# filodb/FiloDB

Measured on NVIDIA H100. Metric: samples/s scanned+aggregated (rate over 10M series); % HBM roofline, higher is better.
Workload: dtype f64

## Files before the change

### filodb_b200/csrc/capi.cu

```cuda
#include "../../include/filo_b200.h"
#include "kernels.h"
#include "host_util.h"
#include "scan_tile_layout.h"
#include "scan_wp_layout.h"
#include <cub/cub.cuh>
#include <algorithm>
#include <atomic>
#include <chrono>
#include <cmath>
#include <cstdio>
#include <cstdlib>
#include <cstring>
#include <mutex>
#include <string>
#include <thread>
#include <vector>

using namespace filo;

struct filo_ctx {
  int device = 0;
  filo_cfg cfg{};
  cudaStream_t stream = nullptr;
  int sm_count = 132;
  size_t max_smem_optin = 0;
  std::mutex err_mu;
  std::string err;
  double fn_args[2] = {0.0, 0.0};
  struct ErrSlot { int* h = nullptr; cudaEvent_t ev = nullptr; bool pending = false; };
  std::mutex errslot_mu;
  ErrSlot errslots[16];
  int errslot_next = 0;
  struct ScanSlot {
    uint8_t* h_in = nullptr; size_t h_in_cap = 0;
    int64_t* h_off = nullptr; size_t h_off_cap = 0;
    uint8_t* d_in = nullptr; size_t d_in_cap = 0;
    int64_t* d_off = nullptr; size_t d_off_cap = 0;
    double* d_out = nullptr; size_t d_out_cap = 0;
    void* h_sink = nullptr;
    void* h_gch = nullptr; size_t h_gch_cap = 0;
    void* d_gch = nullptr; size_t d_gch_cap = 0;
    void* h_gs = nullptr; size_t h_gs_cap = 0;
    void* d_gs = nullptr; size_t d_gs_cap = 0;
    uint8_t* d_stage = nullptr; size_t d_stage_cap = 0;
    cudaStream_t stream = nullptr; cudaEvent_t done = nullptr;
  };
  std::mutex scan_mu;
  static constexpr int MAX_SCAN_SLOTS = 8;
  ScanSlot scan[MAX_SCAN_SLOTS];
  struct HostRange { uintptr_t base; size_t bytes; };
  std::vector<HostRange> ranges;
};

struct filo_table {
  int64_t n_series = 0, n_chunks = 0, n_samples = 0, arena_bytes = 0, algorithmic_bytes = 0;
  int32_t max_rows = 0, max_chunks = 0, schema_flags = 0;
  uint32_t max_rec_bytes = 0;
  bool any_nonconst_ts = true;
  bool any_drop = true;
  uint8_t* d_arena = nullptr;
  int64_t* d_rec_off = nullptr;
  int32_t n_groups = 1;
  bool grouped = false;
  int32_t* d_order = nullptr;
  int64_t* d_group_start = nullptr;
  int64_t* d_gis = nullptr;
  int64_t* d_item_begin = nullptr;
  int64_t n_items = 0;
  int seg = 1;
  bool hist = false, hist_exp = false; int hist_nb = 0;
  bool hist_simple = false;
  std::vector<double> hist_tops; double* d_hist_tops = nullptr;
};

static thread_local std::string tl_err;

static int32_t fail(filo_ctx* ctx, int32_t code, const std::string& msg) {
  tl_err = msg;
  if (ctx) { std::lock_guard<std::mutex> g(ctx->err_mu); ctx->err = msg; }
  return code;
}
#define CUDA_TRY(ctx, expr) do { cudaError_t _e = (expr); if (_e != cudaSuccess) \
  return fail(ctx, _e == cudaErrorMemoryAllocation ? FILO_ERR_OOM : FILO_ERR_CUDA, std::string(#expr) + ": " + cudaGetErrorString(_e)); } while (0)

extern "C" {

int32_t filo_last_error(filo_ctx* ctx, char* buf, int32_t len) {
  std::string m;
  if (ctx) { std::lock_guard<std::mutex> g(ctx->err_mu); m = ctx->err; } else m = tl_err;
  if (buf && len > 0) { int n = std::min<int>(len - 1, (int)m.size()); std::memcpy(buf, m.data(), n); buf[n] = 0; }
  return (int32_t)m.size();
}

int32_t filo_ctx_create(int32_t device, const filo_cfg* cfg, filo_ctx** out) {
  if (!out) return fail(nullptr, FILO_ERR_INVALID_ARG, "out is null");
  int ndev = 0;
  cudaError_t e = cudaGetDeviceCount(&ndev);
  if (e != cudaSuccess || ndev == 0)
    return fail(nullptr, FILO_ERR_CUDA, std::string("no CUDA device (no CPU fallback exists): ") + cudaGetErrorString(e));
  if (device < 0 || device >= ndev) return fail(nullptr, FILO_ERR_INVALID_ARG, "bad device ordinal");
  CUDA_TRY(nullptr, cudaSetDevice(device));
  auto* c = new filo_ctx();
  c->device = device;
  if (cfg) c->cfg = *cfg; else { c->cfg.inclusive_range = 1; c->cfg.group_by_cardinality_limit = 0; c->cfg.min_step_ms = 0; c->cfg.max_data_per_shard_query = 0; }
  cudaDeviceProp p; CUDA_TRY(nullptr, cudaGetDeviceProperties(&p, device));
  c->sm_count = p.multiProcessorCount;
  c->max_smem_optin = p.sharedMemPerBlockOptin;
  CUDA_TRY(nullptr, cudaStreamCreateWithFlags(&c->stream, cudaStreamNonBlocking));
  {
    cudaMemPool_t pool = nullptr;
    if (cudaDeviceGetDefaultMemPool(&pool, device) == cudaSuccess && pool) {
      uint64_t thr = ~0ull;
      cudaMemPoolSetAttribute(pool, cudaMemPoolAttrReleaseThreshold, &thr);
    }
    cudaGetLastError();
  }
  *out = c;
  return FILO_OK;
}

int32_t filo_ctx_set_fn_args(filo_ctx* ctx, double arg0, double arg1) {
  if (!ctx) return fail(nullptr, FILO_ERR_INVALID_ARG, "ctx is null");
  ctx->fn_args[0] = arg0; ctx->fn_args[1] = arg1;
  return FILO_OK;
}

void filo_ctx_destroy(filo_ctx* ctx) {
  if (!ctx) return;
  cudaSetDevice(ctx->device);
  if (ctx->stream) cudaStreamDestroy(ctx->stream);
  for (auto& sl : ctx->errslots) { if (sl.ev) { cudaEventSynchronize(sl.ev); cudaEventDestroy(sl.ev); } if (sl.h) cudaFreeHost(sl.h); }
  for (auto& r : ctx->ranges) cudaHostUnregister((void*)r.base);
  for (auto& sl : ctx->scan) {
    if (sl.stream) cudaStreamSynchronize(sl.stream);
    cudaFreeHost(sl.h_in); cudaFreeHost(sl.h_off); cudaFreeHost(sl.h_sink); cudaFree(sl.d_in); cudaFree(sl.d_off); cudaFree(sl.d_out);
    cudaFreeHost(sl.h_gch); cudaFreeHost(sl.h_gs); cudaFree(sl.d_gch); cudaFree(sl.d_gs); cudaFree(sl.d_stage);
    if (sl.done) cudaEventDestroy(sl.done);
    if (sl.stream) cudaStreamDestroy(sl.stream);
  }
  delete ctx;
}

void filo_table_free(filo_ctx* ctx, filo_table* t) {
  if (!t) return;
  if (ctx) cudaSetDevice(ctx->device);
  cudaFree(t->d_arena); cudaFree(t->d_rec_off); cudaFree(t->d_order); cudaFree(t->d_group_start);
  cudaFree(t->d_gis); cudaFree(t->d_item_begin); cudaFree(t->d_hist_tops);
  delete t;
}

int32_t filo_table_get_info(const filo_table* t, filo_table_info* o) {
  if (!t || !o) return FILO_ERR_INVALID_ARG;
  o->n_series = t->n_series; o->n_chunks = t->n_chunks; o->n_samples = t->n_samples; o->arena_bytes = t->arena_bytes;
  o->algorithmic_bytes = t->algorithmic_bytes; o->max_rows_per_series = t->max_rows; o->max_chunks_per_series = t->max_chunks;
  o->n_groups = t->n_groups; o->schema_flags = t->schema_flags; o->hist_buckets = t->hist ? t->hist_nb : 0; o->reserved = 0;
  return FILO_OK;
}

int32_t filo_num_windows(int64_t start, int64_t step, int64_t end) {
  if (step <= 0) step = 1;
  if (end < start) return 1;
  return (int32_t)((end - start) / step) + 1;
}

}

static bool hist_v2_enabled() { const char* e = getenv("FILO_HIST_V2"); return !(e && e[0] == '0'); }

static int32_t build_groups_new(filo_ctx* ctx, filo_table* t, const int32_t* d_group_ids, int32_t n_groups);
static int32_t build_groups(filo_ctx* ctx, filo_table* t, const int32_t* d_group_ids , int32_t n_groups) {
  int32_t* o_order = t->d_order; int64_t* o_gs = t->d_group_start; int64_t* o_gis = t->d_gis; int64_t* o_ib = t->d_item_begin;
  const int32_t o_ng = t->n_groups; const bool o_grouped = t->grouped; const int64_t o_items = t->n_items; const int o_seg = t->seg;
  t->d_order = nullptr; t->d_group_start = t->d_gis = t->d_item_begin = nullptr;
  const int32_t rc = build_groups_new(ctx, t, d_group_ids, n_groups);
  if (rc != FILO_OK) {
    cudaFree(t->d_order); cudaFree(t->d_group_start); cudaFree(t->d_gis); cudaFree(t->d_item_begin);
    t->d_order = o_order; t->d_group_start = o_gs; t->d_gis = o_gis; t->d_item_begin = o_ib;
    t->n_groups = o_ng; t->grouped = o_grouped; t->n_items = o_items; t->seg = o_seg;
    return rc;
  }
  cudaFree(o_order); cudaFree(o_gs); cudaFree(o_gis); cudaFree(o_ib);
  return FILO_OK;
}
static int32_t build_groups_new(filo_ctx* ctx, filo_table* t, const int32_t* d_group_ids , int32_t n_groups) {
  cudaStream_t s = ctx->stream;
  const int64_t S = t->n_series;
  if (n_groups <= 0) n_groups = 1;
  t->n_groups = n_groups;
  t->grouped = d_group_ids != nullptr;
  int64_t target_items = (int64_t)ctx->sm_count * 64 * 4;
  int64_t seg_cap = 256;
  if (t->hist && hist_v2_enabled()) { target_items = (int64_t)ctx->sm_count * 2 * 6; seg_cap = 4096; }
  int64_t seg = S / std::max<int64_t>(target_items, 1);
  t->seg = (int)std::min<int64_t>(std::max<int64_t>(seg, 1), seg_cap);
  CUDA_TRY(ctx, cudaMalloc(&t->d_group_start, (size_t)(n_groups + 1) * 8));
  CUDA_TRY(ctx, cudaMalloc(&t->d_gis, (size_t)(n_groups + 1) * 8));
  if (t->grouped && S > 0) {
    int32_t *keys_out = nullptr, *vals_in = nullptr;
    CUDA_TRY(ctx, cudaMalloc(&t->d_order, (size_t)S * 4));
    CUDA_TRY(ctx, cudaMalloc(&keys_out, (size_t)S * 4));
    CUDA_TRY(ctx, cudaMalloc(&vals_in, (size_t)S * 4));
    CUDA_TRY(ctx, launch_iota(vals_in, S, s));
    size_t tmp_bytes = 0;
    int end_bit = 1; while ((1ll << end_bit) < n_groups && end_bit < 31) ++end_bit;
    cub::DeviceRadixSort::SortPairs(nullptr, tmp_bytes, d_group_ids, keys_out, vals_in, t->d_order, (int)S, 0, end_bit, s);
    void* tmp = nullptr; CUDA_TRY(ctx, cudaMalloc(&tmp, tmp_bytes + 16));
    CUDA_TRY(ctx, cub::DeviceRadixSort::SortPairs(tmp, tmp_bytes, d_group_ids, keys_out, vals_in, t->d_order, (int)S, 0, end_bit, s));
    CUDA_TRY(ctx, launch_group_bounds(keys_out, S, n_groups, t->d_group_start, s));
    CUDA_TRY(ctx, cudaStreamSynchronize(s));
    cudaFree(tmp); cudaFree(keys_out); cudaFree(vals_in);
  } else {
    std::vector<int64_t> gs(n_groups + 1, S); gs[0] = 0;
    CUDA_TRY(ctx, cudaMemcpyAsync(t->d_group_start, gs.data(), gs.size() * 8, cudaMemcpyHostToDevice, s));
    CUDA_TRY(ctx, cudaStreamSynchronize(s));
  }
  int64_t* d_cnt = nullptr; CUDA_TRY(ctx, cudaMalloc(&d_cnt, (size_t)(n_groups + 1) * 8));
  CUDA_TRY(ctx, cudaMemsetAsync(d_cnt, 0, (size_t)(n_groups + 1) * 8, s));
  CUDA_TRY(ctx, launch_group_item_count(t->d_group_start, n_groups, t->seg, d_cnt, s));
  size_t tmp_bytes = 0;
  cub::DeviceScan::ExclusiveSum(nullptr, tmp_bytes, d_cnt, t->d_gis, n_groups + 1, s);
  void* tmp = nullptr; CUDA_TRY(ctx, cudaMalloc(&tmp, tmp_bytes + 16));
  CUDA_TRY(ctx, cub::DeviceScan::ExclusiveSum(tmp, tmp_bytes, d_cnt, t->d_gis, n_groups + 1, s));
  int64_t n_items = 0;
  CUDA_TRY(ctx, cudaMemcpyAsync(&n_items, t->d_gis + n_groups, 8, cudaMemcpyDeviceToHost, s));
  CUDA_TRY(ctx, cudaStreamSynchronize(s));
  t->n_items = n_items;
  CUDA_TRY(ctx, cudaMalloc(&t->d_item_begin, (size_t)(n_items + 1) * 8));
  CUDA_TRY(ctx, launch_fill_items(t->d_group_start, t->d_gis, n_groups, t->seg, n_items, S, t->d_item_begin, s));
  CUDA_TRY(ctx, cudaStreamSynchronize(s));
  cudaFree(tmp); cudaFree(d_cnt);
  return FILO_OK;
}

int32_t filo_internal_finish_table(filo_ctx* ctx, filo_table* t, const int32_t* d_group_ids, int32_t n_groups) {
  return build_groups(ctx, t, d_group_ids, n_groups);
}
filo_table* filo_internal_new_table() { return new filo_table(); }
void filo_internal_set_arena(filo_table* t, uint8_t* d_arena, int64_t* d_rec_off, int64_t n_series, int64_t n_chunks, int64_t n_samples,
                             int64_t arena_bytes, int64_t algorithmic_bytes, int32_t max_rows, int32_t max_chunks, int32_t schema_flags) {
  t->d_arena = d_arena; t->d_rec_off = d_rec_off; t->n_series = n_series; t->n_chunks = n_chunks; t->n_samples = n_samples;
  t->arena_bytes = arena_bytes; t->algorithmic_bytes = algorithmic_bytes; t->max_rows = max_rows; t->max_chunks = max_chunks;
  t->schema_flags = schema_flags;
}
void filo_internal_set_layout(filo_table* t, uint32_t max_rec_bytes, bool any_nonconst_ts, bool any_drop) {
  t->max_rec_bytes = max_rec_bytes; t->any_nonconst_ts = any_nonconst_ts; t->any_drop = any_drop;
}
cudaStream_t filo_internal_stream(filo_ctx* ctx) { return ctx->stream; }
int filo_internal_device(filo_ctx* ctx) { return ctx->device; }
int32_t filo_internal_fail(filo_ctx* ctx, int32_t code, const char* msg) { return fail(ctx, code, msg); }

namespace {

struct GatherChunk {
  uint64_t ts_src, val_src;
  int64_t start_time, end_time;
  int32_t num_rows, ts_bytes, val_bytes, val_len;
  int32_t drop_patch, pad;
};
struct GatherSeries { uint32_t rec_bytes, n_chunks, n_rows, flags; int64_t first_chunk; };

struct VecInfo { const uint8_t* p; int32_t total; int32_t len; bool drop_patch; bool drop; bool hist = false; };

inline int32_t rd32(const uint8_t* p) { int32_t v; std::memcpy(&v, p, 4); return v; }
inline int64_t rd64(const uint8_t* p) { int64_t v; std::memcpy(&v, p, 8); return v; }

inline bool inner_ok(const uint8_t* in, int32_t& len, int32_t outer_total) {
  const int32_t inner_bytes = rd32(in);
  if (inner_bytes < 4 || (int64_t)20 + 4 + inner_bytes > outer_total) return false;
  int nbits = in[6] & 0x7f; bool sgn = in[6] & 0x80; int bs = in[7] & 0x3f;
  bool ok = sgn ? (nbits == 32 || nbits == 16 || nbits == 8) : (nbits == 32 || nbits == 16 || nbits == 8 || nbits == 4 || nbits == 2);
  if (!ok) return false;
  len = ((rd32(in) - 4) * 8 + (bs != 0 ? bs - 8 : 0)) / nbits;
  return true;
}

int classify_ts(const uint8_t* v, VecInfo& o) {
  int wire = (uint16_t)(v[4] | (v[5] << 8));
  if (wire == WIRE_MASKED) { v = v + rd32(v + 8); wire = (uint16_t)(v[4] | (v[5] << 8)); if (wire == WIRE_MASKED) return FILO_ERR_CORRUPT_VECTOR; }
  o.p = v; o.total = rd32(v) + 4; o.drop_patch = false; o.drop = false;
  if (o.total < 8 || o.total > (1 << 28)) return FILO_ERR_CORRUPT_VECTOR;
  if (wire == WIRE_DDV_CONST) { if (o.total != 24) return FILO_ERR_CORRUPT_VECTOR; o.len = rd32(v + 8); }
  else if (wire == WIRE_RAW64) o.len = (rd32(v) - 4) / 8;
  else if (wire == WIRE_DDV) { if (o.total < 28 || !inner_ok(v + 20, o.len, o.total)) return FILO_ERR_CORRUPT_VECTOR; }
  else return FILO_ERR_CORRUPT_VECTOR;
  return (o.total >= 8 && o.len >= 0) ? 0 : FILO_ERR_CORRUPT_VECTOR;
}
int classify_val(const uint8_t* v, VecInfo& o) {
  int wire = (uint16_t)(v[4] | (v[5] << 8));
  const bool outer_drop = (v[7] & 0x80) != 0;
  bool masked = false;
  if (wire == WIRE_MASKED) { masked = true; v = v + rd32(v + 8); wire = (uint16_t)(v[4] | (v[5] << 8)); if (wire == WIRE_MASKED) return FILO_ERR_CORRUPT_VECTOR; }
  o.p = v; o.total = rd32(v) + 4; o.drop_patch = masked; o.drop = outer_drop;
  if (o.total < 8 || o.total > (1 << 28)) return FILO_ERR_CORRUPT_VECTOR;
  if (wire == WIRE_RAW64) o.len = (rd32(v) - 4) / 8;
  else if (wire == WIRE_DDV_CONST) { if (o.total != 24) return FILO_ERR_CORRUPT_VECTOR; o.len = rd32(v + 8); }
  else if (wire == WIRE_DDV) { if (o.total < 28 || !inner_ok(v + 20, o.len, o.total)) return FILO_ERR_CORRUPT_VECTOR; }
  else if (wire == WIRE_XOR) {
    o.len = rd32(v + XOR_OFF_N);
    int ng = (uint16_t)(v[12] | (v[13] << 8)), po = (uint16_t)(v[14] | (v[15] << 8));
    if (o.len <= 0 || ng != (o.len - 1 + 7) / 8 || po < 16 + 2 * ng || (po & 7) || po + 8 > o.total) return FILO_ERR_CORRUPT_VECTOR;
  } else if (wire == WIRE_H_SECTDELTA || wire == WIRE_H_SIMPLE) {
    if (masked || o.total < 13) return FILO_ERR_CORRUPT_VECTOR;
    o.len = (uint16_t)(v[6] | (v[7] << 8)); o.drop = false; o.hist = true;
    const int fmt = v[8], defBytes = (uint16_t)(v[9] | (v[10] << 8));
    if (o.len > 0 && (!(fmt == 3 || fmt == 4 || fmt == 5 || fmt == 9) || 11 + defBytes > o.total || (fmt == 9 && defBytes != 16)))
      return (fmt == 8 || fmt == 0x0a || fmt == 0x10 || fmt == 9) ? FILO_ERR_UNSUPPORTED : FILO_ERR_CORRUPT_VECTOR;
  } else if (wire == WIRE_H_EXP_SIMPLE) return FILO_ERR_UNSUPPORTED;
  else return FILO_ERR_CORRUPT_VECTOR;
  return (o.total >= 8 && o.len >= 0) ? 0 : FILO_ERR_CORRUPT_VECTOR;
}

struct SeriesPlan { uint32_t rec_bytes; uint32_t n_chunks; uint32_t n_rows; uint32_t flags; };

struct LoadIn { int64_t n_series; const int32_t* n_chunks; const uint64_t* addrs; const int64_t* chunk_base ; int32_t ts_col, val_col;
                GatherChunk* gc_out = nullptr; int64_t gc_base = 0; const std::vector<filo_ctx::HostRange>* ranges = nullptr;
                int64_t cb0 = 0; };
struct PlanTotals { int64_t chunks = 0, samples = 0, alg = 0; int32_t maxrows = 0, maxch = 0; uint32_t max_rec = 0, f_or = 0, f_and = ~0u;
// ... 155 lines not shown
  CUDA_TRY(ctx, cudaMemcpy(t->d_hist_tops, t->hist_tops.data(), (size_t)nb * 8, cudaMemcpyHostToDevice));
  return FILO_OK;
}
static int32_t filo_load_series_impl(filo_ctx* ctx, int64_t n_series, const int32_t* n_chunks, const uint64_t* addrs,
                                    int32_t ts_col, int32_t val_col, const int32_t* group_ids, int32_t n_groups,
                                    int32_t schema_flags, filo_table** out) {
  if (!ctx || !out || n_series < 0 || (n_series > 0 && (!n_chunks || !addrs)) || ts_col < 0 || val_col < 0)
    return fail(ctx, FILO_ERR_INVALID_ARG, "filo_load_series: bad arguments");
  if (group_ids && n_groups <= 0) return fail(ctx, FILO_ERR_INVALID_ARG, "group_ids given but n_groups <= 0");
  if (group_ids && ctx->cfg.group_by_cardinality_limit > 0 && n_groups > ctx->cfg.group_by_cardinality_limit)
    return fail(ctx, FILO_ERR_QUERY_LIMIT, "Query exceeded group-by cardinality limit");
  CUDA_TRY(ctx, cudaSetDevice(ctx->device));
  std::vector<int64_t> chunk_base((size_t)n_series + 1, 0);
  for (int64_t i = 0; i < n_series; ++i) {
    if (n_chunks[i] < 0) return fail(ctx, FILO_ERR_INVALID_ARG, "negative n_chunks");
    chunk_base[i + 1] = chunk_base[i] + n_chunks[i];
  }
  std::vector<SeriesPlan> plan((size_t)n_series);
  const LoadIn in{n_series, n_chunks, addrs, chunk_base.data(), ts_col, val_col};
  PlanTotals tot; int64_t err_series = -1;
  if (const int err_code = plan_all(in, plan, tot, err_series)) {
    const char* what = err_code == FILO_ERR_UNSUPPORTED ? "chunks of a series are not in increasing time order (unsupported on the device path)"
                                                       : "CorruptVector: unknown or inconsistent BinaryVector wire format";
    return fail(ctx, err_code, std::string(what) + " at series " + std::to_string(err_series));
  }
  std::vector<int64_t> rec_off((size_t)n_series + 1, 0);
  for (int64_t i = 0; i < n_series; ++i) rec_off[i + 1] = rec_off[i] + plan[i].rec_bytes;
  const int64_t arena_bytes = rec_off[n_series];
  if (ctx->cfg.max_data_per_shard_query > 0 && tot.alg > ctx->cfg.max_data_per_shard_query)
    return fail(ctx, FILO_ERR_QUERY_LIMIT, "raw data bytes scanned exceeds max-data-per-shard-query");
  if (tot.hist_def && tot.any_scalar) return fail(ctx, FILO_ERR_UNSUPPORTED, "histogram and scalar value vectors in one table");
  if (tot.hist_mismatch) return fail(ctx, FILO_ERR_UNSUPPORTED, "histogram bucket schemes differ inside the table (unsupported on the device path)");
  struct LoadGuard {
    filo_table* t = nullptr; uint8_t* d_arena = nullptr; int64_t* d_rec_off = nullptr; uint8_t* slab[2] = {nullptr, nullptr}; cudaEvent_t ev[2] = {nullptr, nullptr};
    bool owns_table = true;
    ~LoadGuard() {
      for (int b = 0; b < 2; ++b) { if (ev[b]) { cudaEventSynchronize(ev[b]); cudaEventDestroy(ev[b]); } if (slab[b]) cudaFreeHost(slab[b]); }
      if (owns_table) { cudaFree(d_arena); cudaFree(d_rec_off); delete t; }
    }
  } lg;
  lg.t = new filo_table();
  filo_table*& t = lg.t; uint8_t*& d_arena = lg.d_arena; int64_t*& d_rec_off = lg.d_rec_off;
  CUDA_TRY(ctx, cudaMalloc(&d_arena, (size_t)arena_bytes + 64));
  CUDA_TRY(ctx, cudaMalloc(&d_rec_off, (size_t)(n_series + 1) * 8));
  CUDA_TRY(ctx, cudaMemsetAsync(d_arena + arena_bytes, 0, 64, ctx->stream));
  CUDA_TRY(ctx, cudaMemcpyAsync(d_rec_off, rec_off.data(), (size_t)(n_series + 1) * 8, cudaMemcpyHostToDevice, ctx->stream));
  const size_t SLAB = std::min<size_t>((size_t)256 << 20, std::max<size_t>((size_t)arena_bytes, 1 << 16));
  uint8_t** slab = lg.slab; cudaEvent_t* ev = lg.ev;
  for (int b = 0; b < 2; ++b) { CUDA_TRY(ctx, cudaHostAlloc(&slab[b], SLAB + (1 << 20), cudaHostAllocDefault)); CUDA_TRY(ctx, cudaEventCreateWithFlags(&ev[b], cudaEventDisableTiming)); }
  int64_t s0 = 0; int which = 0;
  while (s0 < n_series) {
    int64_t s1 = s0; const int64_t base = rec_off[s0];
    while (s1 < n_series && (size_t)(rec_off[s1 + 1] - base) <= SLAB) ++s1;
    if (s1 == s0) {
      const size_t need = (size_t)plan[s0].rec_bytes;
      CUDA_TRY(ctx, cudaEventSynchronize(ev[which]));
      cudaFreeHost(slab[which]); slab[which] = nullptr;
      CUDA_TRY(ctx, cudaHostAlloc(&slab[which], need + (1 << 20), cudaHostAllocDefault)); s1 = s0 + 1;
    }
    CUDA_TRY(ctx, cudaEventSynchronize(ev[which]));
    uint8_t* dst0 = slab[which];
    host_pool().run(s1 - s0, [&](int, int64_t b, int64_t e) {
      for (int64_t ii = b; ii < e; ++ii) { const int64_t i = s0 + ii; fill_record(in, i, plan[(size_t)i], dst0 + (rec_off[i] - base)); }
    });
    CUDA_TRY(ctx, cudaMemcpyAsync(d_arena + base, dst0, (size_t)(rec_off[s1] - base), cudaMemcpyHostToDevice, ctx->stream));
    CUDA_TRY(ctx, cudaEventRecord(ev[which], ctx->stream));
    which ^= 1; s0 = s1;
  }
  CUDA_TRY(ctx, cudaStreamSynchronize(ctx->stream));
  lg.owns_table = false;
  filo_internal_set_arena(t, d_arena, d_rec_off, n_series, tot.chunks, tot.samples, arena_bytes + (n_series + 1) * 8, tot.alg, tot.maxrows, tot.maxch, schema_flags);
  filo_internal_set_layout(t, tot.max_rec, n_series > 0 && !(tot.f_and & REC_ALL_TS_CONST), (tot.f_or & REC_ANY_DROP) != 0);
  if (tot.hist_def) {
    const int32_t rch = filo_internal_set_hist(ctx, t, tot.hist_def);
    if (rch != FILO_OK) { filo_table_free(ctx, t); return rch; }
    t->hist_simple = tot.hist_simple;
  }
  int32_t* d_gid = nullptr;
  if (group_ids && n_series > 0) {
    for (int64_t i = 0; i < n_series; ++i) if (group_ids[i] < 0 || group_ids[i] >= n_groups) { filo_table_free(ctx, t); return fail(ctx, FILO_ERR_INVALID_ARG, "group id out of range"); }
    CUDA_TRY(ctx, cudaMalloc(&d_gid, (size_t)n_series * 4));
    CUDA_TRY(ctx, cudaMemcpy(d_gid, group_ids, (size_t)n_series * 4, cudaMemcpyHostToDevice));
  }
  int32_t rc = build_groups(ctx, t, d_gid, group_ids ? n_groups : 1);
  cudaFree(d_gid);
  if (rc) { filo_table_free(ctx, t); return rc; }
  *out = t;
  return FILO_OK;
}
extern "C" int32_t filo_load_series(filo_ctx* ctx, int64_t n_series, const int32_t* n_chunks, const uint64_t* addrs,
                                    int32_t ts_col, int32_t val_col, const int32_t* group_ids, int32_t n_groups,
                                    int32_t schema_flags, filo_table** out) {
  try { return filo_load_series_impl(ctx, n_series, n_chunks, addrs, ts_col, val_col, group_ids, n_groups, schema_flags, out); }
  catch (const std::bad_alloc&) { return fail(ctx, FILO_ERR_OOM, "filo_load_series: host allocation failed"); }
  catch (const std::exception& e) { return fail(ctx, FILO_ERR_INVALID_ARG, std::string("filo_load_series: ") + e.what()); }
}

extern "C" int32_t filo_table_set_groups(filo_ctx* ctx, filo_table* t, const int32_t* group_ids, int32_t n_groups) {
  if (!ctx || !t) return fail(ctx, FILO_ERR_INVALID_ARG, "null");
  CUDA_TRY(ctx, cudaSetDevice(ctx->device));
  if (group_ids && ctx->cfg.group_by_cardinality_limit > 0 && n_groups > ctx->cfg.group_by_cardinality_limit)
    return fail(ctx, FILO_ERR_QUERY_LIMIT, "Query exceeded group-by cardinality limit");
  int32_t* d_gid = nullptr;
  if (group_ids && t->n_series > 0) {
    for (int64_t i = 0; i < t->n_series; ++i) if (group_ids[i] < 0 || group_ids[i] >= n_groups) return fail(ctx, FILO_ERR_INVALID_ARG, "group id out of range");
    CUDA_TRY(ctx, cudaMalloc(&d_gid, (size_t)t->n_series * 4));
    CUDA_TRY(ctx, cudaMemcpy(d_gid, group_ids, (size_t)t->n_series * 4, cudaMemcpyHostToDevice));
  }
  int32_t rc = build_groups(ctx, t, d_gid, group_ids ? n_groups : 1);
  cudaFree(d_gid);
  return rc;
}

extern "C" int64_t filo_table_read_record(filo_ctx* ctx, const filo_table* t, int64_t series, uint8_t* out, int64_t cap) {
  if (!ctx || !t || series < 0 || series >= t->n_series) return fail(ctx, FILO_ERR_INVALID_ARG, "bad series");
  cudaSetDevice(ctx->device);
  int64_t off[2];
  if (cudaMemcpy(off, t->d_rec_off + series, 16, cudaMemcpyDeviceToHost) != cudaSuccess) return fail(ctx, FILO_ERR_CUDA, "read rec_off");
  int64_t n = off[1] - off[0];
  if (n > cap) return -n;
  if (cudaMemcpy(out, t->d_arena + off[0], (size_t)n, cudaMemcpyDeviceToHost) != cudaSuccess) return fail(ctx, FILO_ERR_CUDA, "read record");
  return n;
}

namespace {
__device__ __forceinline__ uint32_t rec_used_vectors(const uint8_t* r) {
  const RecordHeader h = *reinterpret_cast<const RecordHeader*>(r);
  const uint32_t v0 = (uint32_t)sizeof(RecordHeader) + 32u * h.n_chunks;
  if (h.n_chunks == 0) return 0;
  const ChunkEntry& e = reinterpret_cast<const ChunkEntry*>(r + sizeof(RecordHeader))[h.n_chunks - 1];
  const uint32_t vt = *reinterpret_cast<const uint32_t*>(r + e.val_off) + 4u;
  return align_up(e.val_off + vt, 8) - v0;
}
__global__ void append_size_kernel(const uint8_t* __restrict__ ar_o, const int64_t* __restrict__ off_o, const uint8_t* __restrict__ ar_d, const int64_t* __restrict__ off_d,
                                   int64_t n, int64_t* __restrict__ sz) {
  const int64_t i = (int64_t)blockIdx.x * blockDim.x + threadIdx.x;
  if (i < n) {
    const uint8_t* ro = ar_o + off_o[i]; const uint8_t* rd = ar_d + off_d[i];
    const uint32_t nn = reinterpret_cast<const RecordHeader*>(ro)->n_chunks + reinterpret_cast<const RecordHeader*>(rd)->n_chunks;
    sz[i] = (int64_t)align_up((uint32_t)sizeof(RecordHeader) + 32u * nn + rec_used_vectors(ro) + rec_used_vectors(rd), 16);
  }
  if (i == n) sz[i] = 0;
}
__global__ void __launch_bounds__(256) append_merge_kernel(const uint8_t* __restrict__ ar_o, const int64_t* __restrict__ off_o, const uint8_t* __restrict__ ar_d,
                                                           const int64_t* __restrict__ off_d, const int64_t* __restrict__ off_n, int64_t n,
                                                           uint8_t* __restrict__ ar_n, unsigned int* __restrict__ stats) {
  const int lane = threadIdx.x & 31;
  const int64_t i = ((int64_t)blockIdx.x * blockDim.x + threadIdx.x) >> 5;
  if (i >= n) return;
  const uint8_t* ro = ar_o + off_o[i]; const uint8_t* rd = ar_d + off_d[i]; uint8_t* rn = ar_n + off_n[i];
  const RecordHeader ho = *reinterpret_cast<const RecordHeader*>(ro), hd = *reinterpret_cast<const RecordHeader*>(rd);
  const uint32_t no = ho.n_chunks, nd = hd.n_chunks, nn = no + nd;
  const uint32_t vo0 = (uint32_t)sizeof(RecordHeader) + 32u * no, vd0 = (uint32_t)sizeof(RecordHeader) + 32u * nd, vn0 = (uint32_t)sizeof(RecordHeader) + 32u * nn;
  const uint32_t Lo = rec_used_vectors(ro), Ld = rec_used_vectors(rd);
  const uint32_t rec_bytes = align_up(vn0 + Lo + Ld, 16);
  if (lane == 0) {
    RecordHeader hn; hn.rec_bytes = rec_bytes; hn.n_chunks = nn; hn.n_rows = ho.n_rows + hd.n_rows;
    hn.flags = ((ho.flags & hd.flags) & REC_ALL_TS_CONST) | ((ho.flags | hd.flags) & ~REC_ALL_TS_CONST);
    *reinterpret_cast<RecordHeader*>(rn) = hn;
    atomicMax(&stats[0], hn.rec_bytes); atomicMax(&stats[1], hn.n_rows); atomicMax(&stats[2], nn);
    if (no && nd) {
      const ChunkEntry& lo = reinterpret_cast<const ChunkEntry*>(ro + sizeof(RecordHeader))[no - 1];
      const ChunkEntry& fd = reinterpret_cast<const ChunkEntry*>(rd + sizeof(RecordHeader))[0];
      if (fd.start_time < lo.start_time || fd.end_time < lo.end_time) atomicAdd(&stats[3], 1u);
    }
    if ((vn0 + Lo + Ld) & 8u) *reinterpret_cast<uint64_t*>(rn + vn0 + Lo + Ld) = 0ull;
  }
  for (uint32_t c = lane; c < nn; c += 32) {
    ChunkEntry e;
    if (c < no) { e = reinterpret_cast<const ChunkEntry*>(ro + sizeof(RecordHeader))[c]; e.ts_off += 32u * nd; e.val_off += 32u * nd; }
    else { e = reinterpret_cast<const ChunkEntry*>(rd + sizeof(RecordHeader))[c - no]; e.ts_off += 32u * no + Lo; e.val_off += 32u * no + Lo; e.row_base += ho.n_rows; }
    reinterpret_cast<ChunkEntry*>(rn + sizeof(RecordHeader))[c] = e;
  }
  const uint64_t* so = reinterpret_cast<const uint64_t*>(ro + vo0); uint64_t* dn = reinterpret_cast<uint64_t*>(rn + vn0);
  for (uint32_t q = lane; q < Lo / 8; q += 32) dn[q] = so[q];
  const uint64_t* sd = reinterpret_cast<const uint64_t*>(rd + vd0); dn = reinterpret_cast<uint64_t*>(rn + vn0 + Lo);
  for (uint32_t q = lane; q < Ld / 8; q += 32) dn[q] = sd[q];
}
}

static int32_t filo_table_append_impl(filo_ctx* ctx, filo_table* t, const int32_t* n_chunks, const uint64_t* chunk_info_addrs, int32_t ts_col, int32_t val_col) {
  if (!ctx || !t || !n_chunks || !chunk_info_addrs) return fail(ctx, FILO_ERR_INVALID_ARG, "filo_table_append: null argument");
  if (t->hist) return fail(ctx, FILO_ERR_UNSUPPORTED, "filo_table_append: histogram tables are rebuilt with filo_load_series");
  const int64_t S = t->n_series;
  filo_table* d = nullptr;
  { const int32_t rc = filo_load_series(ctx, S, n_chunks, chunk_info_addrs, ts_col, val_col, nullptr, 0, t->schema_flags, &d); if (rc != FILO_OK) return rc; }
  struct FreeT { filo_ctx* c; filo_table* t; ~FreeT() { filo_table_free(c, t); } } guard{ctx, d};
  if (d->hist) return fail(ctx, FILO_ERR_UNSUPPORTED, "filo_table_append: histogram vectors");
  CUDA_TRY(ctx, cudaSetDevice(ctx->device));
  cudaStream_t s = ctx->stream;
  int64_t *d_sz = nullptr, *d_off = nullptr; unsigned int* d_stats = nullptr; void* tmp = nullptr; uint8_t* d_arena = nullptr;
  struct FreeD { std::vector<void*> p; ~FreeD() { for (void* x : p) cudaFree(x); } } tmps;
  CUDA_TRY(ctx, cudaMalloc(&d_sz, (size_t)(S + 1) * 8)); tmps.p.push_back(d_sz);
  CUDA_TRY(ctx, cudaMalloc(&d_off, (size_t)(S + 1) * 8));
  CUDA_TRY(ctx, cudaMalloc(&d_stats, 16)); tmps.p.push_back(d_stats);
  CUDA_TRY(ctx, cudaMemsetAsync(d_stats, 0, 16, s));
  append_size_kernel<<<(unsigned)((S + 1 + 255) / 256), 256, 0, s>>>(t->d_arena, t->d_rec_off, d->d_arena, d->d_rec_off, S, d_sz);
  size_t tmp_bytes = 0;
  cub::DeviceScan::ExclusiveSum(nullptr, tmp_bytes, d_sz, d_off, (int)(S + 1), s);
  if (cudaMalloc(&tmp, tmp_bytes + 16) != cudaSuccess) { cudaFree(d_off); return fail(ctx, FILO_ERR_OOM, "filo_table_append: scan storage"); }
  tmps.p.push_back(tmp);
  if (cub::DeviceScan::ExclusiveSum(tmp, tmp_bytes, d_sz, d_off, (int)(S + 1), s) != cudaSuccess) { cudaFree(d_off); return fail(ctx, FILO_ERR_CUDA, "filo_table_append: scan"); }
  int64_t arena_bytes = 0;
  if (cudaMemcpyAsync(&arena_bytes, d_off + S, 8, cudaMemcpyDeviceToHost, s) != cudaSuccess || cudaStreamSynchronize(s) != cudaSuccess) { cudaFree(d_off); return fail(ctx, FILO_ERR_CUDA, "filo_table_append: sizes"); }
  if (cudaMalloc(&d_arena, (size_t)arena_bytes + 64) != cudaSuccess) { cudaFree(d_off); return fail(ctx, FILO_ERR_OOM, "filo_table_append: the new arena does not fit beside the old one"); }
  cudaMemsetAsync(d_arena + arena_bytes, 0, 64, s);
  if (S > 0) append_merge_kernel<<<(unsigned)((S * 32 + 255) / 256), 256, 0, s>>>(t->d_arena, t->d_rec_off, d->d_arena, d->d_rec_off, d_off, S, d_arena, d_stats);
  unsigned int st[4] = {0, 0, 0, 0};
  cudaError_t e = cudaGetLastError();
  if (e == cudaSuccess) e = cudaMemcpyAsync(st, d_stats, 16, cudaMemcpyDeviceToHost, s);
  if (e == cudaSuccess) e = cudaStreamSynchronize(s);
  if (e != cudaSuccess) { cudaFree(d_off); cudaFree(d_arena); return fail(ctx, FILO_ERR_CUDA, std::string("filo_table_append: ") + cudaGetErrorString(e)); }
  if (st[3]) { cudaFree(d_off); cudaFree(d_arena); return fail(ctx, FILO_ERR_UNSUPPORTED, "filo_table_append: new chunks must follow the resident ones in time (unsupported on the device path)"); }
  cudaFree(t->d_arena); cudaFree(t->d_rec_off);
  t->d_arena = d_arena; t->d_rec_off = d_off;
  t->n_chunks += d->n_chunks; t->n_samples += d->n_samples; t->algorithmic_bytes += d->algorithmic_bytes;
  t->arena_bytes = arena_bytes + (S + 1) * 8;
  t->max_rec_bytes = st[0]; t->max_rows = (int32_t)st[1]; t->max_chunks = (int32_t)st[2];
  t->any_nonconst_ts = t->any_nonconst_ts || (d->n_chunks > 0 && d->any_nonconst_ts); t->any_drop = t->any_drop || d->any_drop;
  return FILO_OK;
}
extern "C" int32_t filo_table_append(filo_ctx* ctx, filo_table* t, const int32_t* n_chunks, const uint64_t* chunk_info_addrs, int32_t ts_col, int32_t val_col) {
  try { return filo_table_append_impl(ctx, t, n_chunks, chunk_info_addrs, ts_col, val_col); }
  catch (const std::bad_alloc&) { return fail(ctx, FILO_ERR_OOM, "filo_table_append: host allocation failed"); }
  catch (const std::exception& e) { return fail(ctx, FILO_ERR_INVALID_ARG, std::string("filo_table_append: ") + e.what()); }
}

extern "C" int64_t filo_table_read_arena(filo_ctx* ctx, const filo_table* t, int64_t first, int64_t n, uint8_t* out, int64_t cap,
                                         int64_t* rec_off_out) {
  if (!ctx || !t || first < 0 || n < 0 || first + n > t->n_series || !rec_off_out) return fail(ctx, FILO_ERR_INVALID_ARG, "bad range");
  cudaSetDevice(ctx->device);
  if (cudaMemcpy(rec_off_out, t->d_rec_off + first, (size_t)(n + 1) * 8, cudaMemcpyDeviceToHost) != cudaSuccess)
    return fail(ctx, FILO_ERR_CUDA, "read rec_off");
  const int64_t base = rec_off_out[0], bytes = rec_off_out[n] - base;
  for (int64_t i = 0; i <= n; ++i) rec_off_out[i] -= base;
  if (bytes > cap || !out) return -bytes;
  if (bytes > 0 && cudaMemcpy(out, t->d_arena + base, (size_t)bytes, cudaMemcpyDeviceToHost) != cudaSuccess)
    return fail(ctx, FILO_ERR_CUDA, "read arena");
  return bytes;
}

namespace {
struct Temp {
  cudaStream_t s; std::vector<void*> ptrs;
  explicit Temp(cudaStream_t st) : s(st) {}
  ~Temp() { for (void* p : ptrs) cudaFreeAsync(p, s); }
  cudaError_t alloc(void** p, size_t bytes) { cudaError_t e = cudaMallocAsync(p, bytes ? bytes : 16, s); if (e == cudaSuccess) ptrs.push_back(*p); return e; }
};
}

namespace {
struct AsyncSink { int herr[4]; unsigned long long hc[2]; int64_t launches; };
}
static int32_t query_device_impl(filo_ctx* ctx, const filo_table* t, int32_t fn, int64_t start, int64_t step, int64_t end, int64_t window,
                                 int32_t agg, int32_t k, int32_t flags, void* d_out_values, void* d_out_aux, void* cuda_stream,
                                 filo_stats* stats, AsyncSink* sink);
extern "C" int32_t filo_query_device(filo_ctx* ctx, const filo_table* t, int32_t fn, int64_t start, int64_t step, int64_t end, int64_t window,
                                     int32_t agg, int32_t k, int32_t flags, void* d_out_values, void* d_out_aux, void* cuda_stream,
                                     filo_stats* stats) {
  return query_device_impl(ctx, t, fn, start, step, end, window, agg, k, flags, d_out_values, d_out_aux, cuda_stream, stats, nullptr);
}
namespace {
struct EventPair {
  cudaEvent_t e0 = nullptr, e1 = nullptr;
  ~EventPair() { if (e0) cudaEventDestroy(e0); if (e1) cudaEventDestroy(e1); }
};
}
static int32_t report_device_error(filo_ctx* ctx, const int herr[4], int64_t series_base);
static int32_t poll_async_errors(filo_ctx* ctx, bool wait) {
  std::lock_guard<std::mutex> g(ctx->errslot_mu);
  int32_t rc = FILO_OK;
  for (auto& sl : ctx->errslots) {
    if (!sl.pending) continue;
    cudaError_t e = wait ? cudaEventSynchronize(sl.ev) : cudaEventQuery(sl.ev);
    if (e == cudaErrorNotReady) { cudaGetLastError(); continue; }
    sl.pending = false;
    if (e != cudaSuccess) { if (rc == FILO_OK) rc = fail(ctx, FILO_ERR_CUDA, std::string("asynchronous query: ") + cudaGetErrorString(e)); continue; }
    if (sl.h[0] && rc == FILO_OK) rc = report_device_error(ctx, sl.h, 0);
  }
  return rc;
}
static int32_t push_async_error(filo_ctx* ctx, const int* d_err, cudaStream_t s) {
  std::lock_guard<std::mutex> g(ctx->errslot_mu);
  filo_ctx::ErrSlot& sl = ctx->errslots[ctx->errslot_next];
  ctx->errslot_next = (ctx->errslot_next + 1) % 16;
  if (!sl.h) { CUDA_TRY(ctx, cudaMallocHost((void**)&sl.h, 16)); CUDA_TRY(ctx, cudaEventCreateWithFlags(&sl.ev, cudaEventDisableTiming)); }
  if (sl.pending) {
    CUDA_TRY(ctx, cudaEventSynchronize(sl.ev)); sl.pending = false;
    if (sl.h[0]) return report_device_error(ctx, sl.h, 0);
  }
  CUDA_TRY(ctx, cudaMemcpyAsync(sl.h, d_err, 16, cudaMemcpyDeviceToHost, s));
  CUDA_TRY(ctx, cudaEventRecord(sl.ev, s));
  sl.pending = true;
  return FILO_OK;
}
extern "C" int32_t filo_ctx_check(filo_ctx* ctx) {
  if (!ctx) return fail(nullptr, FILO_ERR_INVALID_ARG, "ctx is null");
  return poll_async_errors(ctx, true);
}
static int32_t report_device_error(filo_ctx* ctx, const int herr[4], int64_t series_base) {
  if (herr[0] == 5)
    return fail(ctx, FILO_ERR_UNSUPPORTED, "histogram series with more chunks / sections / rows in range than the device path holds, at series " +
                std::to_string(series_base + ((int64_t)herr[1] | ((int64_t)herr[2] << 31))));
  const char* what = herr[0] == 4 ? "series needs more decode scratch than the table statistics promised" : "CorruptVector on device";
  return fail(ctx, FILO_ERR_CORRUPT_VECTOR, std::string(what) + " (code " + std::to_string(herr[0]) + ") at series " +
              std::to_string(series_base + ((int64_t)herr[1] | ((int64_t)herr[2] << 31))));
}
static int32_t query_device_impl(filo_ctx* ctx, const filo_table* t, int32_t fn, int64_t start, int64_t step, int64_t end, int64_t window,
                                 int32_t agg, int32_t k, int32_t flags, void* d_out_values, void* d_out_aux, void* cuda_stream,
                                 filo_stats* stats, AsyncSink* sink) {
  if (!ctx || !t || !d_out_values) return fail(ctx, FILO_ERR_INVALID_ARG, "filo_query: null argument");
  if (fn < FILO_FN_LAST || fn > FILO_FN_PRESENT_OVER_TIME) return fail(ctx, FILO_ERR_INVALID_ARG, "unknown range function");
  if (t->hist) return fail(ctx, FILO_ERR_UNSUPPORTED, "histogram table: use filo_query_hist");
  const bool long_values = (t->schema_flags & FILO_SCHEMA_LONG_VALUES) != 0;
  if (long_values && !fn_long_column_ok(fn)) return fail(ctx, FILO_ERR_UNSUPPORTED, "no chunked range function for this function on a Long column");
  if (fn == FILO_FN_HOLT_WINTERS) {
    if (!(ctx->fn_args[0] >= 0 && ctx->fn_args[0] <= 1)) return fail(ctx, FILO_ERR_INVALID_ARG, "Sf should be in between 0 and 1");
    if (!(ctx->fn_args[1] >= 0 && ctx->fn_args[1] <= 1)) return fail(ctx, FILO_ERR_INVALID_ARG, "tf should be in between 0 and 1");
  }
  if (agg < FILO_AGG_NONE || agg > FILO_AGG_GROUP) return fail(ctx, FILO_ERR_INVALID_ARG, "unknown aggregation operator");
  if (start > end) return fail(ctx, FILO_ERR_INVALID_ARG, "start should be <= end");
  if (!(start == end || step > 0)) return fail(ctx, FILO_ERR_INVALID_ARG, "step should be > 0 for range query");
  if (start < end && step < ctx->cfg.min_step_ms) return fail(ctx, FILO_ERR_BAD_QUERY, "step should be at least min-step");
  const int64_t adjustedStep = step > 0 ? step : step + 1;
  const bool isLast = (fn == FILO_FN_LAST || fn == FILO_FN_TIMESTAMP);
  if (window <= 0) { if (isLast) window = 5 * 60 * 1000 + 1; else return fail(ctx, FILO_ERR_INVALID_ARG, "Need positive window lengths to apply range function"); }
  if ((agg == FILO_AGG_TOPK || agg == FILO_AGG_BOTTOMK) && (k <= 0 || k > FILO_MAX_TOPK)) return fail(ctx, FILO_ERR_INVALID_ARG, "topk/bottomk k must be in [1, 32]");
  if ((agg == FILO_AGG_TOPK || agg == FILO_AGG_BOTTOMK || agg == FILO_AGG_AVG) && !d_out_aux && !(agg == FILO_AGG_AVG && !(flags & FILO_Q_PARTIAL)))
    return fail(ctx, FILO_ERR_INVALID_ARG, "out_aux required");
  if ((flags & FILO_Q_PARTIAL) && agg != FILO_AGG_NONE && agg != FILO_AGG_TOPK && agg != FILO_AGG_BOTTOMK && !d_out_aux)
    return fail(ctx, FILO_ERR_INVALID_ARG, "partial aggregates need out_aux (counts)");
  CUDA_TRY(ctx, cudaSetDevice(ctx->device));
  { const int32_t prc = poll_async_errors(ctx, false); if (prc != FILO_OK) return prc; }
  cudaStream_t s = cuda_stream ? (cudaStream_t)cuda_stream : ctx->stream;
  QueryParams q{};
  q.start = start; q.step = adjustedStep; q.end = end; q.window = window; q.T = filo_num_windows(start, adjustedStep, end);
  q.fn = fn; q.cumulative = (t->schema_flags & FILO_SCHEMA_CUMULATIVE) ? 1 : 0; q.inclusive = ctx->cfg.inclusive_range ? 1 : 0;
  q.long_values = long_values ? 1 : 0; q.p0 = ctx->fn_args[0]; q.p1 = ctx->fn_args[1];
  const bool need_corr = (fn == FILO_FN_RATE || fn == FILO_FN_INCREASE) && q.cumulative;
  const bool fused = (agg != FILO_AGG_NONE && agg != FILO_AGG_TOPK && agg != FILO_AGG_BOTTOMK);
  const bool moments = agg_moments(agg);
  const int scan_op = moments ? AGG_SUM : agg == FILO_AGG_GROUP ? AGG_COUNT : agg;

  Temp tmp(s);
  int* d_err = nullptr; unsigned long long* d_counters = nullptr;
  CUDA_TRY(ctx, tmp.alloc((void**)&d_err, 16)); CUDA_TRY(ctx, tmp.alloc((void**)&d_counters, 16));
  CUDA_TRY(ctx, cudaMemsetAsync(d_err, 0, 16, s)); CUDA_TRY(ctx, cudaMemsetAsync(d_counters, 0, 16, s));
  EventPair evp;
  if (stats) { CUDA_TRY(ctx, cudaEventCreate(&evp.e0)); CUDA_TRY(ctx, cudaEventCreate(&evp.e1)); }
  cudaEvent_t& e0 = evp.e0; cudaEvent_t& e1 = evp.e1;

  const uint32_t acc_bytes = fused ? align_up((uint32_t)q.T * (moments ? 20u : 12u), 128) : 0;
  const bool need_corr2 = need_corr && t->any_drop;
  uint32_t scratch2 = align_up((uint32_t)t->max_chunks * (uint32_t)CHUNK_DESC_BYTES, 16) +
                      ((uint32_t)t->max_rows + (uint32_t)t->max_chunks * 8u) * 8u * (1u + (t->any_nonconst_ts ? 1u : 0u) + (need_corr2 ? 1u : 0u));
  scratch2 = align_up(scratch2 + 16, 128);
  const uint32_t rec_cap = align_up(t->max_rec_bytes + 16, 128);
  const size_t per_warp2 = v2_smem_per_warp(rec_cap, scratch2, acc_bytes);
  const char* force_env = std::getenv("FILO_KERNEL");
  const std::string force = force_env ? force_env : "";
  const size_t smem_cap = std::min<size_t>(ctx->max_smem_optin, 227 * 1024);
  const bool use_v2 = force != "v1" && t->max_rec_bytes > 0 && per_warp2 * FAST_WARPS + 1024 <= smem_cap;
  const int64_t work = fused ? t->n_items : t->n_series;
  int64_t launches = 0;
  uint8_t* gscratch = nullptr;
  ScanLaunch L{t->d_arena, t->d_rec_off, t->n_series, q, nullptr, 0, 0, d_counters, d_err, 1, s};
  uint32_t rec_cap_used = 0;
  if (use_v2) {
    const size_t cta_smem = per_warp2 * FAST_WARPS + 1024;
    const int ctas_per_sm = (int)std::max<size_t>(1, std::min<size_t>(64 / FAST_WARPS, (size_t)(228 * 1024) / cta_smem));
    L.grid = (int)std::max<int64_t>(1, std::min<int64_t>((work + FAST_WARPS - 1) / FAST_WARPS, (int64_t)ctx->sm_count * ctas_per_sm));
    L.scratch_bytes = scratch2; L.use_smem = 1; rec_cap_used = rec_cap;
  } else {
    uint32_t scratch = align_up((uint32_t)t->max_chunks * (uint32_t)CHUNK_DESC_BYTES, 16) + (uint32_t)t->max_rows * 8u * (need_corr ? 3u : 2u);
    scratch = align_up(scratch + 16, 16);
    const size_t cta_smem = (size_t)(scratch + acc_bytes) * SCAN_WARPS;
    const int use_smem = cta_smem <= std::min<size_t>(ctx->max_smem_optin, 200 * 1024);
    int ctas_per_sm = 16;
    if (use_smem) ctas_per_sm = (int)std::max<size_t>(1, std::min<size_t>(16, (size_t)(220 * 1024) / std::max<size_t>(cta_smem + 1024, 1)));
    L.grid = (int)std::max<int64_t>(1, std::min<int64_t>((work + SCAN_WARPS - 1) / SCAN_WARPS, (int64_t)ctx->sm_count * ctas_per_sm));
    if (!use_smem) CUDA_TRY(ctx, tmp.alloc((void**)&gscratch, (size_t)L.grid * SCAN_WARPS * (scratch + acc_bytes)));
    L.gscratch = gscratch; L.scratch_bytes = scratch; L.use_smem = use_smem;
  }
  const int fn_cls = fn_class_of(fn, q.cumulative, q.long_values);
  const uint64_t wrows = (uint64_t)(q.window / q.step) + 1;
  TileSmem TL{};
  bool use_tile = false;
  if (use_v2 && force != "v2" && fn_cls == CLASS_SUM && t->n_series > 0) {
    TL = tile_layout(t->max_rec_bytes, (uint32_t)t->max_rows, (uint32_t)q.T, (uint32_t)std::min<uint64_t>(2 * wrows, 1u << 20) + 16);
    if (((size_t)TL.total + 1024) * 2 > (size_t)228 * 1024) TL = tile_layout(t->max_rec_bytes, (uint32_t)t->max_rows, (uint32_t)q.T, 16);
    use_tile = (size_t)TL.total + 1024 <= smem_cap;
  }
  WpSmem WL{};
  bool use_wp = false;
  if (use_tile && force != "v3" && wrows <= 4096 && t->max_chunks > 0) {
    const bool alias = wp_max_items((uint32_t)t->max_chunks, (uint32_t)q.T, (uint32_t)wrows) <= 64;
    WL = wp_layout(t->max_rec_bytes, (uint32_t)t->max_rows, (uint32_t)t->max_chunks, (uint32_t)q.T, (uint32_t)wrows, alias);
    WL.warps = (uint32_t)std::min<size_t>(smem_cap / WL.per_warp, alias ? WP_MAX_WARPS_ALIAS : WP_MAX_WARPS);
    const WpSmem WL2 = wp_layout(t->max_rec_bytes, (uint32_t)t->max_rows, (uint32_t)t->max_chunks, (uint32_t)q.T, (uint32_t)wrows, alias, true);
    if (smem_cap / WL2.per_warp >= (size_t)WP_MAX_WARPS) { WL = WL2; WL.warps = WP_MAX_WARPS; }
    use_wp = WL.warps >= 4;
  }
  WpCtrSmem WC{};
  bool use_wp_ctr = false;
  if (use_v2 && force != "v2" && force != "v3" && fn_cls == CLASS_COUNTER && t->n_series > 0 && t->max_chunks > 0 &&
      (!fused || q.T <= TILE_AGG_ACC * TILE_THREADS) && wp_ctr_tile_footprint_ok(t->max_rec_bytes, (uint32_t)t->max_rows, (uint32_t)q.T, smem_cap)) {
    WC = wp_ctr_layout(t->max_rec_bytes, (uint32_t)t->max_rows, (uint32_t)t->max_chunks, (uint32_t)q.T, fused, t->any_nonconst_ts, moments);
    const size_t w = std::min<size_t>((smem_cap - sizeof(TileCtrTab) * (TILE_CTR_TABMAX + 1) - 64) / WC.per_warp, WC.tsr != 0 ? 16 : WP_CTR_MAX_WARPS);
    WC.warps = (uint32_t)w; WC.tab = (uint32_t)(WC.per_warp * w);
    use_wp_ctr = w >= 4;
  }
  auto run_per_series = [&](double* outp) -> int32_t {
    if (use_tile || use_wp_ctr) {
      int64_t* d_list = nullptr; unsigned long long* d_cnt = nullptr;
      CUDA_TRY(ctx, tmp.alloc((void**)&d_list, (size_t)t->n_series * 8));
      CUDA_TRY(ctx, tmp.alloc((void**)&d_cnt, 16));
      CUDA_TRY(ctx, cudaMemsetAsync(d_cnt, 0, 16, s));
      ScanLaunch LT = L;
      static const bool dbg = std::getenv("FILO_DEBUG_SYNC") != nullptr;
      if (use_wp) {
        LT.grid = (int)std::max<int64_t>(1, std::min<int64_t>((t->n_series + WL.warps - 1) / WL.warps, (int64_t)ctx->sm_count));
        CUDA_TRY(ctx, launch_scan_wp(LT, outp, WL, d_list, d_cnt));
      } else if (use_wp_ctr) {
        LT.grid = (int)std::max<int64_t>(1, std::min<int64_t>((t->n_series + WC.warps - 1) / WC.warps, (int64_t)ctx->sm_count));
        CUDA_TRY(ctx, launch_scan_wp_ctr(LT, outp, WC, d_list, d_cnt));
      } else {
        const int ctas_per_sm = ((size_t)TL.total + 1024) * 2 <= (size_t)228 * 1024 ? 2 : 1;
        const int64_t n_tiles = (t->n_series + TILE_NS - 1) / TILE_NS;
        LT.grid = (int)std::max<int64_t>(1, std::min<int64_t>(n_tiles, (int64_t)ctx->sm_count * ctas_per_sm));
        if (dbg) { fprintf(stderr, "[filo] tile kernel fn=%d T=%d grid=%d smem=%u pitch=%u\n", fn, q.T, LT.grid, TL.total, TL.vals_pitch); fflush(stderr); }
        CUDA_TRY(ctx, launch_scan_tile(LT, outp, TL, d_list, d_cnt));
      }
      if (dbg) { CUDA_TRY(ctx, cudaStreamSynchronize(s)); fprintf(stderr, "[filo] tile kernel done\n"); fflush(stderr); }
      ScanLaunch LF = L; LF.list = d_list; LF.list_count = d_cnt;
      CUDA_TRY(ctx, launch_scan_series_v2(LF, outp, rec_cap_used));
      if (dbg) { CUDA_TRY(ctx, cudaStreamSynchronize(s)); fprintf(stderr, "[filo] fallback kernel done\n"); fflush(stderr); }
      launches += 2;
    } else {
      CUDA_TRY(ctx, use_v2 ? launch_scan_series_v2(L, outp, rec_cap_used) : launch_scan_series(L, outp));
      launches += 1;
    }
    return FILO_OK;
  };
  if (stats) CUDA_TRY(ctx, cudaEventRecord(e0, s));
  if (agg == FILO_AGG_NONE) {
    { int32_t rc = run_per_series((double*)d_out_values); if (rc) return rc; }
  } else if (!fused) {
    double* per = nullptr;
    CUDA_TRY(ctx, tmp.alloc((void**)&per, (size_t)t->n_series * q.T * 8));
// ... 311 lines not shown
      int32_t rg = FILO_OK;
      if (!use_gather) rg = grow_pinned(ctx, sl.h_in, sl.h_in_cap, B.bytes + 64);
      else {
        rg = grow_pinned(ctx, sl.h_gch, sl.h_gch_cap, (size_t)(B.chunks + 1) * sizeof(GatherChunk));
        if (!rg) rg = grow_device(ctx, sl.d_gch, sl.d_gch_cap, (size_t)(B.chunks + 1) * sizeof(GatherChunk));
        if (!rg) rg = grow_pinned(ctx, sl.h_gs, sl.h_gs_cap, (size_t)(nb + 1) * sizeof(GatherSeries));
        if (!rg) rg = grow_device(ctx, sl.d_gs, sl.d_gs_cap, (size_t)(nb + 1) * sizeof(GatherSeries));
      }
      if (!rg) rg = grow_pinned(ctx, sl.h_off, sl.h_off_cap, (size_t)(nb + 1) * 8);
      if (!rg) rg = grow_device(ctx, sl.d_in, sl.d_in_cap, B.bytes + 64);
      if (!rg) rg = grow_device(ctx, sl.d_off, sl.d_off_cap, (size_t)(nb + 1) * 8);
      if (!rg) rg = grow_device(ctx, sl.d_out, sl.d_out_cap, (size_t)nb * (size_t)std::max(T, 1) * 8);
      if (rg) { rc = rg; break; }
    }
    if (trace_path) {
      TraceRow tr{nb, B.bytes, ms_since(t_begin), {nullptr, nullptr, nullptr, nullptr}};
      for (auto& e : tr.ev) cudaEventCreate(&e);
      if (!trace_t0) { cudaEventCreate(&trace_t0); cudaEventRecord(trace_t0, sl.stream); }
      cudaEventRecord(tr.ev[0], sl.stream);
      trace.push_back(tr);
    }
    const auto t_f0 = now();
    sl.h_off[0] = 0;
    for (int64_t j = 0; j < nb; ++j) sl.h_off[j + 1] = sl.h_off[j] + plan[(size_t)(B.s0 + j - c0)].rec_bytes;
    cudaError_t ce = cudaSuccess;
    if (use_gather) {
      GatherSeries* gs = reinterpret_cast<GatherSeries*>(sl.h_gs); GatherChunk* gc = reinterpret_cast<GatherChunk*>(sl.h_gch);
      int64_t cb = 0;
      for (int64_t j = 0; j < nb; ++j) { const SeriesPlan& p = plan[(size_t)(B.s0 + j - c0)]; gs[j] = GatherSeries{p.rec_bytes, p.n_chunks, p.n_rows, p.flags, cb}; cb += p.n_chunks; }
      std::atomic<uint64_t> span_lo{~0ull}, span_hi{0};
      host_pool().run(nb, [&](int, int64_t b, int64_t e) {
        uint64_t lo = ~0ull, hi = 0;
        for (int64_t j = b; j < e; ++j) {
          const int64_t i = B.s0 + j; GatherChunk* o = gc + gs[j].first_chunk;
          const GatherChunk* src = gc_walk.data() + (chunk_base[(size_t)(i - c0)] - in.gc_base);
          for (uint32_t jj = 0; jj < gs[j].n_chunks; ++jj) {
            const GatherChunk g = src[jj];
            *o++ = g;
            lo = std::min(lo, std::min(g.ts_src, g.val_src));
            hi = std::max(hi, std::max(g.ts_src + (uint64_t)g.ts_bytes, g.val_src + (uint64_t)g.val_bytes));
          }
        }
        uint64_t cur = span_lo.load(); while (lo < cur && !span_lo.compare_exchange_weak(cur, lo)) {}
        cur = span_hi.load(); while (hi > cur && !span_hi.compare_exchange_weak(cur, hi)) {}
      });
      t_fill += ms_since(t_f0);
      int64_t rebase = 0;
      {
        static const bool no_span = [] { const char* e = std::getenv("FILO_SCAN_SPAN"); return e && e[0] == '0'; }();
        const uint64_t lo = span_lo.load() & ~(uint64_t)15, hi = span_hi.load();
        if (!no_span && hi > lo && (hi - lo) <= (uint64_t)B.bytes + (uint64_t)B.bytes / 2 + (1u << 20) && in_ranges(reinterpret_cast<const uint8_t*>((uintptr_t)lo), (size_t)(hi - lo))) {
          if (int32_t rcg = grow_device(ctx, sl.d_stage, sl.d_stage_cap, (size_t)(hi - lo) + 64)) return rcg;
          ce = cudaMemcpyAsync(sl.d_stage, reinterpret_cast<const void*>((uintptr_t)lo), (size_t)(hi - lo), cudaMemcpyHostToDevice, sl.stream);
          rebase = (int64_t)((uint64_t)(uintptr_t)sl.d_stage - lo);
        }
      }
      if (ce == cudaSuccess)
      ce = cudaMemcpyAsync(sl.d_gs, sl.h_gs, (size_t)nb * sizeof(GatherSeries), cudaMemcpyHostToDevice, sl.stream);
      if (ce == cudaSuccess) ce = cudaMemcpyAsync(sl.d_gch, sl.h_gch, (size_t)B.chunks * sizeof(GatherChunk), cudaMemcpyHostToDevice, sl.stream);
      if (ce == cudaSuccess) ce = cudaMemcpyAsync(sl.d_off, sl.h_off, (size_t)(nb + 1) * 8, cudaMemcpyHostToDevice, sl.stream);
      if (ce == cudaSuccess) {
        const int grid = (int)std::max<int64_t>(1, std::min<int64_t>((nb + 7) / 8, (int64_t)ctx->sm_count * 8));
        gather_records_kernel<<<grid, 256, 0, sl.stream>>>(reinterpret_cast<const GatherSeries*>(sl.d_gs), reinterpret_cast<const GatherChunk*>(sl.d_gch),
                                                           sl.d_off, nb, sl.d_in, rebase);
        ce = cudaGetLastError();
      }
      if (ce == cudaSuccess) ce = cudaMemsetAsync(sl.d_in + B.bytes, 0, 64, sl.stream);
    } else {
      host_pool().run(nb, [&](int, int64_t b, int64_t e) {
        for (int64_t j = b; j < e; ++j) fill_record(in, B.s0 + j, plan[(size_t)(B.s0 + j - c0)], sl.h_in + sl.h_off[j]);
      });
      std::memset(sl.h_in + B.bytes, 0, 64);
      t_fill += ms_since(t_f0);
      ce = cudaMemcpyAsync(sl.d_in, sl.h_in, B.bytes + 64, cudaMemcpyHostToDevice, sl.stream);
      if (ce == cudaSuccess) ce = cudaMemcpyAsync(sl.d_off, sl.h_off, (size_t)(nb + 1) * 8, cudaMemcpyHostToDevice, sl.stream);
    }
    const auto t_e0 = now();
    if (ce != cudaSuccess) { rc = fail(ctx, FILO_ERR_CUDA, std::string("scan H2D: ") + cudaGetErrorString(ce)); break; }
    if (trace_path) cudaEventRecord(trace.back().ev[1], sl.stream);
    filo_table view;
    view.n_series = nb; view.d_arena = sl.d_in; view.d_rec_off = sl.d_off; view.max_rows = tot.maxrows; view.max_chunks = tot.maxch;
    view.max_rec_bytes = tot.max_rec; view.any_nonconst_ts = !(tot.f_and & REC_ALL_TS_CONST); view.any_drop = (tot.f_or & REC_ANY_DROP) != 0;
    view.schema_flags = schema_flags; view.n_groups = 1; view.grouped = false;
    rc = query_device_impl(ctx, &view, fn, start, step, end, window, FILO_AGG_NONE, 0, 0, sl.d_out, nullptr, sl.stream, nullptr,
                           reinterpret_cast<AsyncSink*>(sl.h_sink));
    if (rc != FILO_OK) break;
    if (trace_path) cudaEventRecord(trace.back().ev[2], sl.stream);
    ce = cudaMemcpyAsync(out_values + (size_t)B.s0 * T, sl.d_out, (size_t)nb * T * 8, cudaMemcpyDeviceToHost, sl.stream);
    if (trace_path) cudaEventRecord(trace.back().ev[3], sl.stream);
    if (ce == cudaSuccess) ce = cudaEventRecord(sl.done, sl.stream);
    if (ce != cudaSuccess) { rc = fail(ctx, FILO_ERR_CUDA, std::string("scan D2H: ") + cudaGetErrorString(ce)); break; }
    fl[si].s0 = B.s0;
    t_enq += ms_since(t_e0);
    acc.h2d_bytes += (int64_t)B.bytes + (nb + 1) * 8 + (use_gather ? (int64_t)(nb * sizeof(GatherSeries) + B.chunks * sizeof(GatherChunk)) : 0); acc.d2h_bytes += nb * (int64_t)T * 8;
  }
  }
  for (int i = 0; i < NSLOT; ++i) { const int32_t r2 = retire(i); if (rc == FILO_OK) rc = r2; }
  if (rc != FILO_OK) { for (int i = 0; i < NSLOT; ++i) if (ctx->scan[i].stream) cudaStreamSynchronize(ctx->scan[i].stream); return rc; }
  if (trace_path) {
    if (FILE* f = std::fopen(trace_path, "w")) {
      std::fprintf(f, "batch,series,bytes,host_enqueue_ms,start_ms,h2d_done_ms,kernels_done_ms,d2h_done_ms\n");
      for (size_t i = 0; i < trace.size(); ++i) {
        float t[4] = {0, 0, 0, 0};
        for (int j = 0; j < 4; ++j) cudaEventElapsedTime(&t[j], trace_t0, trace[i].ev[j]);
        std::fprintf(f, "%zu,%lld,%zu,%.3f,%.3f,%.3f,%.3f,%.3f\n", i, (long long)trace[i].nb, trace[i].bytes, trace[i].host_ms, t[0], t[1], t[2], t[3]);
      }
      std::fclose(f);
    }
    for (auto& r : trace) for (auto& e : r.ev) cudaEventDestroy(e);
    if (trace_t0) cudaEventDestroy(trace_t0);
  }
  if (timing) fprintf(stderr, "[filo] scan_series: %lld series, %zu batches, total %.1f ms: plan %.1f, fill %.1f, enqueue %.1f, slot waits %.1f\n",
                      (long long)n_series, n_batches, ms_since(t_begin), t_plan, t_fill, t_enq, t_retire);
  if (stats) *stats = acc;
  return FILO_OK;
}
extern "C" int32_t filo_scan_series(filo_ctx* ctx, int64_t n_series, const int32_t* n_chunks, const uint64_t* addrs,
                                    int32_t ts_col, int32_t val_col, int32_t schema_flags,
                                    int32_t fn, int64_t start, int64_t step, int64_t end, int64_t window,
                                    double* out_values, filo_stats* stats) {
  try { return filo_scan_series_impl(ctx, n_series, n_chunks, addrs, ts_col, val_col, schema_flags, fn, start, step, end, window, out_values, stats); }
  catch (const std::bad_alloc&) { return fail(ctx, FILO_ERR_OOM, "filo_scan_series: host allocation failed"); }
  catch (const std::exception& e) { return fail(ctx, FILO_ERR_INVALID_ARG, std::string("filo_scan_series: ") + e.what()); }
}


static int32_t hist_query_impl(filo_ctx* ctx, const filo_table* t, int32_t fn, int64_t start, int64_t step, int64_t end, int64_t window,
                               int32_t agg, double quantile, double* out_values, double* out_quantile, void* cuda_stream, filo_stats* stats, bool host_out) {
  if (!ctx || !t || (!out_values && !out_quantile)) return fail(ctx, FILO_ERR_INVALID_ARG, "filo_query_hist: null argument");
  if (!t->hist) return fail(ctx, FILO_ERR_INVALID_ARG, "filo_query_hist: not a histogram table");
  if (agg != FILO_AGG_NONE && agg != FILO_AGG_SUM) return fail(ctx, FILO_ERR_UNSUPPORTED, "histogram aggregates: sum only");
  if (!(fn == FILO_FN_RATE || fn == FILO_FN_INCREASE || fn == FILO_FN_SUM_OVER_TIME || fn == FILO_FN_LAST))
    return fail(ctx, FILO_ERR_UNSUPPORTED, "histogram range functions on the device path: rate, increase, sum_over_time, last");
  if (start > end) return fail(ctx, FILO_ERR_INVALID_ARG, "start should be <= end");
  if (!(start == end || step > 0)) return fail(ctx, FILO_ERR_INVALID_ARG, "step should be > 0 for range query");
  if (start < end && step < ctx->cfg.min_step_ms) return fail(ctx, FILO_ERR_BAD_QUERY, "step should be at least min-step");
  const bool last = fn == FILO_FN_LAST;
  if (window <= 0) { if (last) window = 5 * 60 * 1000 + 1; else return fail(ctx, FILO_ERR_INVALID_ARG, "Need positive window lengths to apply range function"); }
  CUDA_TRY(ctx, cudaSetDevice(ctx->device));
  { const int32_t prc = poll_async_errors(ctx, false); if (prc != FILO_OK) return prc; }
  cudaStream_t s = cuda_stream ? (cudaStream_t)cuda_stream : ctx->stream;
  const int64_t adjustedStep = step > 0 ? step : step + 1;
  QueryParams q{};
  q.start = start; q.step = adjustedStep; q.end = end; q.window = window; q.T = filo_num_windows(start, adjustedStep, end);
  q.fn = fn; q.cumulative = (t->schema_flags & FILO_SCHEMA_CUMULATIVE) ? 1 : 0; q.inclusive = ctx->cfg.inclusive_range ? 1 : 0;
  const int nb = t->hist_nb, T = q.T;
  const bool fused = agg == FILO_AGG_SUM;
  const bool pq = !fused && out_quantile;
  const size_t smem = hist_smem_bytes(t->max_rows, nb, T, fused || pq, t->max_rec_bytes);
  const size_t smem2 = hist2_smem_bytes(t->max_rows, nb, t->max_rec_bytes);
  const bool v2 = hist_v2_enabled() && ((q.cumulative && (fn == FILO_FN_RATE || fn == FILO_FN_INCREASE)) || (last && !t->hist_simple)) && T <= 32 * 512 && nb <= 64 &&
                  smem2 + 1024 <= std::min<size_t>(ctx->max_smem_optin, 227 * 1024) && (fused || pq || last);
  if (!(v2 && !fused) && smem + 2048 > std::min<size_t>(ctx->max_smem_optin, 227 * 1024))
    return fail(ctx, FILO_ERR_UNSUPPORTED, "histogram query does not fit the device working set (rows x buckets or windows x buckets too large)");
  Temp tmp(s);
  int* d_err = nullptr; unsigned long long* d_counters = nullptr;
  CUDA_TRY(ctx, tmp.alloc((void**)&d_err, 16)); CUDA_TRY(ctx, tmp.alloc((void**)&d_counters, 16));
  CUDA_TRY(ctx, cudaMemsetAsync(d_err, 0, 16, s)); CUDA_TRY(ctx, cudaMemsetAsync(d_counters, 0, 16, s));
  EventPair evp;
  if (stats) { CUDA_TRY(ctx, cudaEventCreate(&evp.e0)); CUDA_TRY(ctx, cudaEventCreate(&evp.e1)); }
  cudaEvent_t& e0 = evp.e0; cudaEvent_t& e1 = evp.e1;
  const int64_t work = fused ? t->n_items : t->n_series;
  ScanLaunch L{t->d_arena, t->d_rec_off, t->n_series, q, nullptr, 0, 0, d_counters, d_err, 1, s};
  const int ctas_per_sm = (int)std::max<size_t>(1, (size_t)(228 * 1024) / (smem + 2048));
  L.grid = (int)std::max<int64_t>(1, std::min<int64_t>(work, (int64_t)ctx->sm_count * ctas_per_sm));
  const int64_t rows = fused ? t->n_groups : t->n_series;
  double *d_out = out_values, *d_q = out_quantile, *pval = nullptr; uint8_t* pany = nullptr;
  if (host_out) {
    if (out_values) CUDA_TRY(ctx, tmp.alloc((void**)&d_out, (size_t)rows * T * nb * 8));
    if (out_quantile) CUDA_TRY(ctx, tmp.alloc((void**)&d_q, (size_t)rows * T * 8));
  }
  if (stats) CUDA_TRY(ctx, cudaEventRecord(e0, s));
  if (v2 && !fused) {
    const int cps = (int)std::max<size_t>(1, std::min<size_t>(2, (size_t)(228 * 1024) / (smem2 + 1024)));
    L.grid = (int)std::max<int64_t>(1, std::min<int64_t>(hist2_series_items(t->n_series), (int64_t)ctx->sm_count * cps));
    double* scratch = nullptr;
    if (!out_values) CUDA_TRY(ctx, tmp.alloc((void**)&scratch, (size_t)L.grid * T * nb * 8));
    CUDA_TRY(ctx, launch_hist_scan2_series(L, nb, t->max_rows, t->max_rec_bytes, d_out, d_q, scratch, t->d_hist_tops, quantile, t->hist_exp ? 1 : 0));
  } else if (v2) {
    const int cps = (int)std::max<size_t>(1, std::min<size_t>(2, (size_t)(228 * 1024) / (smem2 + 1024)));
    L.grid = (int)std::max<int64_t>(1, std::min<int64_t>(t->n_items, (int64_t)ctx->sm_count * cps));
    CUDA_TRY(ctx, tmp.alloc((void**)&pval, (size_t)t->n_items * T * nb * 8));
    CUDA_TRY(ctx, tmp.alloc((void**)&pany, (size_t)t->n_items * T + 16));
    CUDA_TRY(ctx, launch_hist_scan2(L, nb, t->max_rows, t->max_rec_bytes, t->grouped ? t->d_order : nullptr, t->d_item_begin, t->n_items, pval, pany));
    CUDA_TRY(ctx, launch_hist_merge2(pval, pany, t->d_gis, t->n_groups, T, nb, t->hist_exp ? 1 : 0, t->d_hist_tops, out_quantile ? quantile : std::nan(""), d_out, d_q, s));
  } else if (fused) {
    CUDA_TRY(ctx, tmp.alloc((void**)&pval, (size_t)t->n_items * T * nb * 8));
    CUDA_TRY(ctx, tmp.alloc((void**)&pany, (size_t)t->n_items * T + 16));
    CUDA_TRY(ctx, launch_hist_scan(L, nb, t->max_rows, t->max_rec_bytes, t->grouped ? t->d_order : nullptr, t->d_item_begin, t->n_items, 1, nullptr, pval, pany));
    CUDA_TRY(ctx, launch_hist_merge(pval, pany, t->d_gis, t->n_groups, T, nb, t->hist_exp ? 1 : 0, t->d_hist_tops, out_quantile ? quantile : std::nan(""), d_out, d_q, s));
  } else {
    CUDA_TRY(ctx, launch_hist_scan(L, nb, t->max_rows, t->max_rec_bytes, nullptr, nullptr, 0, 0, d_out, nullptr, nullptr, t->d_hist_tops, quantile, t->hist_exp ? 1 : 0, d_q));
  }
  if (!stats) return push_async_error(ctx, d_err, s);
  CUDA_TRY(ctx, cudaEventRecord(e1, s));
  int herr[4]; unsigned long long hc[2];
  CUDA_TRY(ctx, cudaMemcpyAsync(herr, d_err, 16, cudaMemcpyDeviceToHost, s));
  CUDA_TRY(ctx, cudaMemcpyAsync(hc, d_counters, 16, cudaMemcpyDeviceToHost, s));
  const size_t d2h = host_out ? (out_values ? (size_t)rows * T * nb * 8 : 0) + (out_quantile ? (size_t)rows * T * 8 : 0) : 0;
  if (host_out && out_values) CUDA_TRY(ctx, cudaMemcpyAsync(out_values, d_out, (size_t)rows * T * nb * 8, cudaMemcpyDeviceToHost, s));
  if (host_out && out_quantile) CUDA_TRY(ctx, cudaMemcpyAsync(out_quantile, d_q, (size_t)rows * T * 8, cudaMemcpyDeviceToHost, s));
  CUDA_TRY(ctx, cudaStreamSynchronize(s));
  float ms = 0; cudaEventElapsedTime(&ms, e0, e1);
  stats->kernel_ns = (int64_t)((double)ms * 1e6); stats->samples_scanned = (int64_t)hc[0]; stats->bytes_scanned = (int64_t)hc[1];
  stats->kernel_launches = fused ? 2 : 1; stats->h2d_bytes = 0; stats->d2h_bytes = (int64_t)d2h;
  if (herr[0]) return report_device_error(ctx, herr, 0);
  return FILO_OK;
}
extern "C" int32_t filo_query_hist_device(filo_ctx* ctx, const filo_table* t, int32_t fn, int64_t start, int64_t step, int64_t end, int64_t window,
                                          int32_t agg, double quantile, void* d_out_values, void* d_out_quantile, void* cuda_stream, filo_stats* stats) {
  try { return hist_query_impl(ctx, t, fn, start, step, end, window, agg, quantile, (double*)d_out_values, (double*)d_out_quantile, cuda_stream, stats, false); }
  catch (const std::bad_alloc&) { return fail(ctx, FILO_ERR_OOM, "filo_query_hist: host allocation failed"); }
  catch (const std::exception& e) { return fail(ctx, FILO_ERR_INVALID_ARG, std::string("filo_query_hist: ") + e.what()); }
}
extern "C" int32_t filo_query_hist(filo_ctx* ctx, const filo_table* t, int32_t fn, int64_t start, int64_t step, int64_t end, int64_t window,
                                   int32_t agg, double quantile, double* out_values, double* out_quantile, filo_stats* stats) {
  filo_stats st{};
  try { const int32_t rc = hist_query_impl(ctx, t, fn, start, step, end, window, agg, quantile, out_values, out_quantile, nullptr, &st, true);
        if (stats) *stats = st;
        return rc; }
  catch (const std::bad_alloc&) { return fail(ctx, FILO_ERR_OOM, "filo_query_hist: host allocation failed"); }
  catch (const std::exception& e) { return fail(ctx, FILO_ERR_INVALID_ARG, std::string("filo_query_hist: ") + e.what()); }
}

extern "C" int32_t filo_merge_hist_partials(filo_ctx* ctx, const filo_table* t, int32_t n_parts, int32_t n_windows, double quantile,
                                            const void* d_parts, void* d_out_values, void* d_out_quantile, void* cuda_stream) {
  if (!ctx || !t || !d_parts) return fail(ctx, FILO_ERR_INVALID_ARG, "filo_merge_hist_partials: null argument");
  if (!t->hist) return fail(ctx, FILO_ERR_INVALID_ARG, "filo_merge_hist_partials: not a histogram table");
  if (n_parts < 1 || n_windows < 1) return fail(ctx, FILO_ERR_INVALID_ARG, "filo_merge_hist_partials: n_parts and n_windows must be >= 1");
  double* d_q = quantile == quantile ? (double*)d_out_quantile : nullptr;
  if (!d_out_values && !d_q) return fail(ctx, FILO_ERR_INVALID_ARG, "filo_merge_hist_partials: no output (values NULL, and quantile NaN or its output NULL)");
  if (t->hist_nb > 64) return fail(ctx, FILO_ERR_UNSUPPORTED, "filo_merge_hist_partials: more than 64 buckets");
  CUDA_TRY(ctx, cudaSetDevice(ctx->device));
  { const int32_t prc = poll_async_errors(ctx, false); if (prc != FILO_OK) return prc; }
  cudaStream_t s = cuda_stream ? (cudaStream_t)cuda_stream : ctx->stream;
  CUDA_TRY(ctx, launch_hist_merge_parts((const double*)d_parts, n_parts, (int64_t)t->n_groups * n_windows, t->hist_nb, t->hist_exp ? 1 : 0, t->d_hist_tops,
                                        quantile, (double*)d_out_values, d_q, s));
  return FILO_OK;
}

extern "C" int32_t filo_present_partials(filo_ctx* ctx, int32_t agg, int64_t n, void* d_values, void* d_counts, void* d_out, void* cuda_stream) {
  if (!ctx || !d_values || !d_counts || !d_out || n < 0) return fail(ctx, FILO_ERR_INVALID_ARG, "filo_present_partials: bad argument");
  CUDA_TRY(ctx, cudaSetDevice(ctx->device));
  cudaStream_t s = cuda_stream ? (cudaStream_t)cuda_stream : ctx->stream;
  if (n > 0) CUDA_TRY(ctx, launch_present(agg, n, (const double*)d_values, (const int64_t*)d_counts, (double*)d_out, s));
  return FILO_OK;
// ... 2 lines not shown
```

### filodb_b200/csrc/kernels.h

```cpp
#pragma once
#include <cuda_runtime.h>
#include <stdint.h>
#include "filo_record.h"

namespace filo {

constexpr int SCAN_WARPS = 4;
constexpr int FAST_WARPS = 4;
constexpr int FAST_MIN_CTAS = 4;
constexpr int CHUNK_DESC_BYTES = 144;
constexpr int FILO_MAX_TOPK = 32;
enum { AGG_NONE = 0, AGG_SUM = 1, AGG_AVG = 2, AGG_MIN = 3, AGG_MAX = 4, AGG_COUNT = 5, AGG_TOPK = 6, AGG_BOTTOMK = 7,
       AGG_STDDEV = 8, AGG_STDVAR = 9, AGG_GROUP = 10 };
__host__ __device__ inline bool agg_moments(int agg_op) { return agg_op == AGG_STDDEV || agg_op == AGG_STDVAR; }
template <bool ON, typename T> struct MomOnly { T v; };
template <typename T> struct MomOnly<false, T> {};

struct QueryParams;

}
#include "scan_params.h"
#include "scan_tile_layout.h"
namespace filo {

struct ScanLaunch {
  const uint8_t* arena; const int64_t* rec_off; int64_t n_series;
  QueryParams q;
  uint8_t* gscratch; uint32_t scratch_bytes; int use_smem;
  unsigned long long* d_counters; int* d_err;
  int grid; cudaStream_t stream;
  const int64_t* list = nullptr; const unsigned long long* list_count = nullptr;
};

cudaError_t launch_scan_series(const ScanLaunch& L, double* out);
cudaError_t launch_scan_agg(const ScanLaunch& L, const int32_t* order, const int64_t* item_begin, int64_t n_items, int agg_op,
                            double* pval, uint32_t* pcnt, uint32_t acc_bytes);
cudaError_t launch_scan_series_v2(const ScanLaunch& L, double* out, uint32_t rec_cap);
cudaError_t launch_scan_agg_v2(const ScanLaunch& L, const int32_t* order, const int64_t* item_begin, int64_t n_items, int agg_op,
                               double* pval, uint32_t* pcnt, uint32_t acc_bytes, uint32_t rec_cap, bool moments = false);
size_t v2_smem_per_warp(uint32_t rec_cap, uint32_t scratch_bytes, uint32_t acc_bytes);
cudaError_t launch_scan_tile(const ScanLaunch& L, double* out, const TileSmem& T, int64_t* fallback_list, unsigned long long* fallback_count);
cudaError_t launch_scan_tile_agg(const ScanLaunch& L, const TileSmem& T, const int32_t* order, const int64_t* item_begin, int64_t n_items, int agg_op,
                                 double* pval, uint32_t* pcnt, int64_t* fallback_list, unsigned long long* fallback_count, bool moments = false);
cudaError_t launch_merge_partials(const double* pval, const uint32_t* pcnt, const int64_t* gis, int n_groups, int T, int agg_op,
                                  int partial_out, double* out_val, int64_t* out_cnt, cudaStream_t s);
cudaError_t launch_present(int agg_op, int64_t n, const double* vals, const int64_t* cnts, double* out, cudaStream_t s);
cudaError_t launch_topk(const double* per_series, const int32_t* order, const int64_t* group_start, int n_groups, int T, int k, int bottom,
                        double* out_val, int64_t* out_id, cudaStream_t s);
struct WpSmem;
cudaError_t launch_scan_wp(const ScanLaunch& L, double* out, const WpSmem& W, int64_t* fallback_list, unsigned long long* fallback_count);
struct WpCtrSmem;
cudaError_t launch_scan_wp_ctr(const ScanLaunch& L, double* out, const WpCtrSmem& W, int64_t* fallback_list, unsigned long long* fallback_count);
cudaError_t launch_scan_wp_ctr_agg(const ScanLaunch& L, const WpCtrSmem& W, const int32_t* order, const int64_t* item_begin, int64_t n_items, int agg_op,
                                   double* pval, uint32_t* pcnt, int64_t* fallback_list, unsigned long long* fallback_count, bool moments = false);
size_t hist_smem_bytes(int max_rows, int nb, int T, bool agg, uint32_t max_rec);
cudaError_t launch_hist_scan(const ScanLaunch& L, int nb, int max_rows, uint32_t max_rec, const int32_t* order, const int64_t* item_begin, int64_t n_items, int agg,
                             double* out, double* pval, uint8_t* pany, const double* tops = nullptr, double qtl = 0.0, int exp_buckets = 0, double* out_q = nullptr);
cudaError_t launch_hist_merge(const double* pval, const uint8_t* pany, const int64_t* gis, int n_groups, int T, int nb, int exp_buckets, const double* tops, double q,
                              double* out_values, double* out_q, cudaStream_t s);
size_t hist2_smem_bytes(int max_rows, int nb, uint32_t max_rec);
cudaError_t launch_hist_scan2(const ScanLaunch& L, int nb, int max_rows, uint32_t max_rec, const int32_t* order, const int64_t* item_begin, int64_t n_items,
                              double* pval, uint8_t* pany);
int64_t hist2_series_items(int64_t n_series);
cudaError_t launch_hist_scan2_series(const ScanLaunch& L, int nb, int max_rows, uint32_t max_rec, double* out_values, double* out_q, double* scratch,
                                     const double* tops, double qtl, int exp_buckets);
cudaError_t launch_hist_merge2(const double* pval, const uint8_t* pany, const int64_t* gis, int n_groups, int T, int nb, int exp_buckets, const double* tops, double q,
                               double* out_values, double* out_q, cudaStream_t s);
cudaError_t launch_hist_merge_parts(const double* parts, int n_parts, int64_t n_cells, int nb, int exp_buckets, const double* tops, double q,
                                    double* out_values, double* out_q, cudaStream_t s);
cudaError_t launch_iota(int32_t* a, int64_t n, cudaStream_t s);
cudaError_t launch_group_bounds(const int32_t* sorted_keys, int64_t n, int n_groups, int64_t* group_start, cudaStream_t s);
cudaError_t launch_group_item_count(const int64_t* group_start, int n_groups, int seg, int64_t* cnt, cudaStream_t s);
cudaError_t launch_fill_items(const int64_t* group_start, const int64_t* gis, int n_groups, int seg, int64_t n_items, int64_t n_series,
                              int64_t* item_begin, cudaStream_t s);

}
```

### filodb_b200/csrc/scan_kernels.cu

```cuda
#include <cuda_runtime.h>
#include <stdint.h>
#define FILO_DEV_ERR_TS_WIRE 1
#define FILO_DEV_ERR_VAL_WIRE 2
#define FILO_DEV_ERR_EMPTY 3
#define FILO_DEV_ERR_SCRATCH 4
#include "scan_device.cuh"
#include "kernels.h"
#include "scan_fast.cuh"
#include "scan_tile.cuh"
#include "scan_wp.cuh"
#include "scan_wp_ctr.cuh"

namespace filo {

__device__ __forceinline__ void report_error(int* d_err, int code, int64_t series) {
  if (atomicCAS(&d_err[0], 0, code) == 0) { d_err[1] = (int)(series & 0x7fffffff); d_err[2] = (int)(series >> 31); }
}

__device__ __forceinline__ int resolve_series(const uint8_t* rec, const QueryParams& q, uint8_t* scratch, uint32_t scratch_bytes,
                                              bool need_corrected, int lane, int& err, int64_t& rows_scanned, int64_t& bytes_scanned) {
  const RecordHeader* h = reinterpret_cast<const RecordHeader*>(rec);
  const ChunkEntry* E = reinterpret_cast<const ChunkEntry*>(rec + sizeof(RecordHeader));
  const int nch = (int)h->n_chunks;
  const int64_t t1 = q.start - q.window, t2 = q.end;
  int cLo = 0; while (cLo < nch && E[cLo].end_time < t1) ++cLo;
  int cHi = cLo; while (cHi < nch && E[cHi].start_time <= t2) ++cHi;
  if (t1 > t2) cHi = cLo;
  const int n = cHi - cLo;
  err = 0;
  if (n <= 0) return 0;
  ChunkDesc* D = reinterpret_cast<ChunkDesc*>(scratch);
  ScratchCursor sc; sc.p = scratch + align_up((uint32_t)n * (uint32_t)sizeof(ChunkDesc), 16);
  uint32_t need = (uint32_t)(sc.p - scratch) + (uint32_t)h->n_rows * 8u * (need_corrected ? 3u : 2u);
  if (need > scratch_bytes) { err = FILO_DEV_ERR_SCRATCH; return 0; }
  for (int c = 0; c < n; ++c) {
    int e = resolve_chunk(rec, &E[cLo + c], &D[c], sc, need_corrected, lane, false, q.long_values != 0);
    if (e) { err = e; return 0; }
  }
  if (lane == 0) {
    const int64_t lastEnd = q.start + (int64_t)(q.T - 1) * q.step;
    int f = 0; while (f < n - 1 && D[f].end_time < lastEnd) ++f;
    for (int c = 0; c <= f; ++c) {
      rows_scanned += D[c].num_rows;
      bytes_scanned += (int64_t)ld32(rec + E[cLo + c].ts_off) + 4 + (int64_t)ld32(rec + E[cLo + c].val_off) + 4;
    }
  }
  return n;
}

__global__ void __launch_bounds__(SCAN_WARPS * 32)
scan_series_kernel(const uint8_t* __restrict__ arena, const int64_t* __restrict__ rec_off, int64_t n_series,
                   QueryParams q, double* __restrict__ out,
                   uint8_t* gscratch, uint32_t scratch_bytes, int use_smem,
                   unsigned long long* d_counters, int* d_err) {
  extern __shared__ __align__(128) uint8_t smem[];
  const int warp = threadIdx.x >> 5, lane = threadIdx.x & 31;
  const int64_t gw = (int64_t)blockIdx.x * SCAN_WARPS + warp, nw = (int64_t)gridDim.x * SCAN_WARPS;
  uint8_t* scratch = use_smem ? smem + (size_t)warp * scratch_bytes : gscratch + (size_t)gw * scratch_bytes;
  const int fn = q.fn;
  const bool need_corrected = ((fn == FN_RATE || fn == FN_INCREASE) && q.cumulative);
  int64_t rows = 0, bytes = 0;
  for (int64_t i = gw; i < n_series; i += nw) {
    const uint8_t* rec = arena + rec_off[i];
    int err;
    const int n = resolve_series(rec, q, scratch, scratch_bytes, need_corrected, lane, err, rows, bytes);
    if (err) { if (lane == 0) report_error(d_err, err, i); continue; }
    const ChunkDesc* D = reinterpret_cast<const ChunkDesc*>(scratch);
    double* o = out + (size_t)i * q.T;
    for (int k = lane; k < q.T; k += 32) o[k] = eval_window(D, 0, n, q, k);
    __syncwarp();
  }
  if (lane == 0 && (rows | bytes)) { atomicAdd(&d_counters[0], (unsigned long long)rows); atomicAdd(&d_counters[1], (unsigned long long)bytes); }
}

__global__ void __launch_bounds__(SCAN_WARPS * 32)
scan_agg_kernel(const uint8_t* __restrict__ arena, const int64_t* __restrict__ rec_off, const int32_t* __restrict__ order,
                const int64_t* __restrict__ item_begin, int64_t n_items,
                QueryParams q, int agg_op, double* __restrict__ pval, uint32_t* __restrict__ pcnt,
                uint8_t* gscratch, uint32_t scratch_bytes, uint32_t acc_bytes, int use_smem,
                unsigned long long* d_counters, int* d_err) {
  extern __shared__ __align__(128) uint8_t smem[];
  const int warp = threadIdx.x >> 5, lane = threadIdx.x & 31;
  const int64_t gw = (int64_t)blockIdx.x * SCAN_WARPS + warp, nw = (int64_t)gridDim.x * SCAN_WARPS;
// ... 301 lines not shown
  cudaError_t e = cudaMemcpyFromSymbol(out16, g_tile_prof, sizeof(unsigned long long) * 16);
  if (e == cudaSuccess && reset) { unsigned long long z[16] = {}; e = cudaMemcpyToSymbol(g_tile_prof, z, sizeof z); }
  return (int)e;
}
#endif
#ifdef FILO_WP_PROF
extern "C" int filo_debug_wp_prof(unsigned long long* out16, int reset) {
  cudaError_t e = cudaMemcpyFromSymbol(out16, g_wp_prof, sizeof(unsigned long long) * 16);
  if (e == cudaSuccess && reset) { unsigned long long z[16] = {}; e = cudaMemcpyToSymbol(g_wp_prof, z, sizeof z); }
  return (int)e;
}
#endif
template <int CLS>
static cudaError_t launch_series_v2_cls(const ScanLaunch& L, double* out, uint32_t rec_cap, size_t smem) {
  cudaError_t e = cudaFuncSetAttribute(scan_series_kernel_v2<CLS>, cudaFuncAttributeMaxDynamicSharedMemorySize, (int)smem);
  if (e != cudaSuccess) return e;
  scan_series_kernel_v2<CLS><<<L.grid, FAST_WARPS * 32, smem, L.stream>>>(L.arena, L.rec_off, L.n_series, L.q, out, rec_cap, L.scratch_bytes,
                                                                           L.d_counters, L.d_err, L.list, L.list_count);
  return cudaGetLastError();
}
cudaError_t launch_scan_series_v2(const ScanLaunch& L, double* out, uint32_t rec_cap) {
  const size_t smem = (size_t)(WARP_HDR_BYTES + rec_cap + STAGE_BYTES + L.scratch_bytes) * FAST_WARPS;
  switch (fn_class_of(L.q.fn, L.q.cumulative, L.q.long_values)) {
    case CLASS_SUM: return launch_series_v2_cls<CLASS_SUM>(L, out, rec_cap, smem);
    case CLASS_MINMAX: return launch_series_v2_cls<CLASS_MINMAX>(L, out, rec_cap, smem);
    case CLASS_COUNTER: return launch_series_v2_cls<CLASS_COUNTER>(L, out, rec_cap, smem);
    default: return launch_series_v2_cls<CLASS_POINT>(L, out, rec_cap, smem);
  }
}
template <int CLS, bool MOM>
static cudaError_t launch_agg_v2_cls(const ScanLaunch& L, const int32_t* order, const int64_t* item_begin, int64_t n_items, int agg_op,
                                     double* pval, uint32_t* pcnt, uint32_t acc_bytes, uint32_t rec_cap, size_t smem) {
  cudaError_t e = cudaFuncSetAttribute(scan_agg_kernel_v2<CLS, MOM>, cudaFuncAttributeMaxDynamicSharedMemorySize, (int)smem);
  if (e != cudaSuccess) return e;
  scan_agg_kernel_v2<CLS, MOM><<<L.grid, FAST_WARPS * 32, smem, L.stream>>>(L.arena, L.rec_off, order, item_begin, n_items, L.q, agg_op, pval, pcnt,
                                                                             rec_cap, L.scratch_bytes, acc_bytes, L.d_counters, L.d_err, L.list, L.list_count);
  return cudaGetLastError();
}
template <bool MOM>
static cudaError_t launch_agg_v2_any(const ScanLaunch& L, const int32_t* order, const int64_t* item_begin, int64_t n_items, int agg_op,
                                     double* pval, uint32_t* pcnt, uint32_t acc_bytes, uint32_t rec_cap, size_t smem) {
  switch (fn_class_of(L.q.fn, L.q.cumulative, L.q.long_values)) {
    case CLASS_SUM: return launch_agg_v2_cls<CLASS_SUM, MOM>(L, order, item_begin, n_items, agg_op, pval, pcnt, acc_bytes, rec_cap, smem);
    case CLASS_MINMAX: return launch_agg_v2_cls<CLASS_MINMAX, MOM>(L, order, item_begin, n_items, agg_op, pval, pcnt, acc_bytes, rec_cap, smem);
    case CLASS_COUNTER: return launch_agg_v2_cls<CLASS_COUNTER, MOM>(L, order, item_begin, n_items, agg_op, pval, pcnt, acc_bytes, rec_cap, smem);
    default: return launch_agg_v2_cls<CLASS_POINT, MOM>(L, order, item_begin, n_items, agg_op, pval, pcnt, acc_bytes, rec_cap, smem);
  }
}
cudaError_t launch_scan_agg_v2(const ScanLaunch& L, const int32_t* order, const int64_t* item_begin, int64_t n_items, int agg_op,
                               double* pval, uint32_t* pcnt, uint32_t acc_bytes, uint32_t rec_cap, bool moments) {
  const size_t smem = (size_t)(WARP_HDR_BYTES + rec_cap + STAGE_BYTES + acc_bytes + L.scratch_bytes) * FAST_WARPS;
  return moments ? launch_agg_v2_any<true>(L, order, item_begin, n_items, agg_op, pval, pcnt, acc_bytes, rec_cap, smem)
                 : launch_agg_v2_any<false>(L, order, item_begin, n_items, agg_op, pval, pcnt, acc_bytes, rec_cap, smem);
}
struct TileAggArgs { const int32_t* order; const int64_t* item_begin; int64_t n_items; int agg_op; double* pval; uint32_t* pcnt; };
template <int FN, bool AGG, bool MOM>
static cudaError_t launch_tile_fn(const ScanLaunch& L, double* out, const TileSmem& T, int64_t* fallback_list, unsigned long long* fallback_count,
                                  const TileAggArgs& A) {
  cudaError_t e = cudaFuncSetAttribute(scan_tile_kernel<FN, AGG, MOM>, cudaFuncAttributeMaxDynamicSharedMemorySize, (int)T.total);
  if (e != cudaSuccess) return e;
  scan_tile_kernel<FN, AGG, MOM><<<L.grid, TILE_LAUNCH_THREADS, T.total, L.stream>>>(L.arena, L.rec_off, L.n_series, L.q, out, T, fallback_list, fallback_count,
      L.d_counters, L.d_err, A.order, A.item_begin, A.n_items, A.agg_op, A.pval, A.pcnt);
  return cudaGetLastError();
}
template <bool AGG, bool MOM = false>
static cudaError_t launch_tile_any(const ScanLaunch& L, double* out, const TileSmem& T, int64_t* fallback_list, unsigned long long* fallback_count,
                                   const TileAggArgs& A) {
  switch (L.q.fn) {
    case FN_RATE: return launch_tile_fn<FN_RATE, AGG, MOM>(L, out, T, fallback_list, fallback_count, A);
    case FN_AVG: return launch_tile_fn<FN_AVG, AGG, MOM>(L, out, T, fallback_list, fallback_count, A);
    case FN_COUNT: return launch_tile_fn<FN_COUNT, AGG, MOM>(L, out, T, fallback_list, fallback_count, A);
    default: return launch_tile_fn<FN_SUM, AGG, MOM>(L, out, T, fallback_list, fallback_count, A);
  }
}
cudaError_t launch_scan_tile(const ScanLaunch& L, double* out, const TileSmem& T, int64_t* fallback_list, unsigned long long* fallback_count) {
  return launch_tile_any<false>(L, out, T, fallback_list, fallback_count, TileAggArgs{nullptr, nullptr, 0, 0, nullptr, nullptr});
}
cudaError_t launch_scan_tile_agg(const ScanLaunch& L, const TileSmem& T, const int32_t* order, const int64_t* item_begin, int64_t n_items, int agg_op,
                                 double* pval, uint32_t* pcnt, int64_t* fallback_list, unsigned long long* fallback_count, bool moments) {
  const TileAggArgs A{order, item_begin, n_items, agg_op, pval, pcnt};
  return moments ? launch_tile_any<true, true>(L, nullptr, T, fallback_list, fallback_count, A)
                 : launch_tile_any<true>(L, nullptr, T, fallback_list, fallback_count, A);
}
template <int FN, int NW>
static cudaError_t launch_wp_nw(const ScanLaunch& L, double* out, const WpSmem& W, int64_t* fallback_list, unsigned long long* fallback_count) {
  const size_t smem = (size_t)W.per_warp * W.warps;
  cudaError_t e = cudaFuncSetAttribute(scan_wp_sum_kernel<FN, NW>, cudaFuncAttributeMaxDynamicSharedMemorySize, (int)smem);
  if (e != cudaSuccess) return e;
  scan_wp_sum_kernel<FN, NW><<<L.grid, W.warps * 32, smem, L.stream>>>(L.arena, L.rec_off, L.n_series, L.q, out, W, fallback_list, fallback_count, L.d_counters, L.d_err);
  return cudaGetLastError();
}
template <int FN>
static cudaError_t launch_wp_fn(const ScanLaunch& L, double* out, const WpSmem& W, int64_t* fallback_list, unsigned long long* fallback_count) {
  if (W.warps <= (uint32_t)WP_MAX_WARPS) return launch_wp_nw<FN, WP_MAX_WARPS>(L, out, W, fallback_list, fallback_count);
  return launch_wp_nw<FN, WP_MAX_WARPS_ALIAS>(L, out, W, fallback_list, fallback_count);
}
cudaError_t launch_scan_wp(const ScanLaunch& L, double* out, const WpSmem& W, int64_t* fallback_list, unsigned long long* fallback_count) {
  switch (L.q.fn) {
    case FN_RATE: return launch_wp_fn<FN_RATE>(L, out, W, fallback_list, fallback_count);
    case FN_AVG: return launch_wp_fn<FN_AVG>(L, out, W, fallback_list, fallback_count);
    case FN_COUNT: return launch_wp_fn<FN_COUNT>(L, out, W, fallback_list, fallback_count);
    default: return launch_wp_fn<FN_SUM>(L, out, W, fallback_list, fallback_count);
  }
}
template <int FN, bool AGG, int NW, bool IRR, bool MOM>
static cudaError_t launch_wp_ctr_nw(const ScanLaunch& L, double* out, const WpCtrSmem& W, int64_t* fallback_list, unsigned long long* fallback_count,
                                    const TileAggArgs& A) {
  const size_t smem = (size_t)W.per_warp * W.warps + sizeof(TileCtrTab) * (TILE_CTR_TABMAX + 1);
  cudaError_t e = cudaFuncSetAttribute(scan_wp_ctr_kernel<FN, AGG, NW, IRR, MOM>, cudaFuncAttributeMaxDynamicSharedMemorySize, (int)smem);
  if (e != cudaSuccess) return e;
  scan_wp_ctr_kernel<FN, AGG, NW, IRR, MOM><<<L.grid, W.warps * 32, smem, L.stream>>>(L.arena, L.rec_off, L.n_series, L.q, out, W, fallback_list, fallback_count,
      L.d_counters, L.d_err, A.order, A.item_begin, A.n_items, A.agg_op, A.pval, A.pcnt);
  return cudaGetLastError();
}
template <int FN, bool AGG, bool MOM>
static cudaError_t launch_wp_ctr_fn(const ScanLaunch& L, double* out, const WpCtrSmem& W, int64_t* fallback_list, unsigned long long* fallback_count, const TileAggArgs& A) {
  if (W.tsr != 0) return launch_wp_ctr_nw<FN, AGG, 16, true, MOM>(L, out, W, fallback_list, fallback_count, A);
  if (W.warps <= 16) return launch_wp_ctr_nw<FN, AGG, 16, false, MOM>(L, out, W, fallback_list, fallback_count, A);
  return launch_wp_ctr_nw<FN, AGG, WP_CTR_MAX_WARPS, false, MOM>(L, out, W, fallback_list, fallback_count, A);
}
template <bool AGG, bool MOM = false>
static cudaError_t launch_wp_ctr_any(const ScanLaunch& L, double* out, const WpCtrSmem& W, int64_t* fallback_list, unsigned long long* fallback_count, const TileAggArgs& A) {
  switch (L.q.fn) {
    case FN_RATE: return launch_wp_ctr_fn<FN_RATE, AGG, MOM>(L, out, W, fallback_list, fallback_count, A);
    case FN_INCREASE: return launch_wp_ctr_fn<FN_INCREASE, AGG, MOM>(L, out, W, fallback_list, fallback_count, A);
    default: return launch_wp_ctr_fn<FN_DELTA, AGG, MOM>(L, out, W, fallback_list, fallback_count, A);
  }
}
cudaError_t launch_scan_wp_ctr(const ScanLaunch& L, double* out, const WpCtrSmem& W, int64_t* fallback_list, unsigned long long* fallback_count) {
  return launch_wp_ctr_any<false>(L, out, W, fallback_list, fallback_count, TileAggArgs{nullptr, nullptr, 0, 0, nullptr, nullptr});
}
cudaError_t launch_scan_wp_ctr_agg(const ScanLaunch& L, const WpCtrSmem& W, const int32_t* order, const int64_t* item_begin, int64_t n_items, int agg_op,
                                   double* pval, uint32_t* pcnt, int64_t* fallback_list, unsigned long long* fallback_count, bool moments) {
  const TileAggArgs A{order, item_begin, n_items, agg_op, pval, pcnt};
  return moments ? launch_wp_ctr_any<true, true>(L, nullptr, W, fallback_list, fallback_count, A)
                 : launch_wp_ctr_any<true>(L, nullptr, W, fallback_list, fallback_count, A);
}
size_t v2_smem_per_warp(uint32_t rec_cap, uint32_t scratch_bytes, uint32_t acc_bytes) { return WARP_HDR_BYTES + (size_t)rec_cap + STAGE_BYTES + acc_bytes + scratch_bytes; }
cudaError_t launch_scan_series(const ScanLaunch& L, double* out) {
  size_t smem = L.use_smem ? (size_t)L.scratch_bytes * SCAN_WARPS : 0;
  if (smem > 48 * 1024) {
    cudaError_t e = cudaFuncSetAttribute(scan_series_kernel, cudaFuncAttributeMaxDynamicSharedMemorySize, (int)smem);
    if (e != cudaSuccess) return e;
  }
  scan_series_kernel<<<L.grid, SCAN_WARPS * 32, smem, L.stream>>>(L.arena, L.rec_off, L.n_series, L.q, out,
      L.gscratch, L.scratch_bytes, L.use_smem, L.d_counters, L.d_err);
  return cudaGetLastError();
}
cudaError_t launch_scan_agg(const ScanLaunch& L, const int32_t* order, const int64_t* item_begin, int64_t n_items, int agg_op,
                            double* pval, uint32_t* pcnt, uint32_t acc_bytes) {
  size_t smem = L.use_smem ? (size_t)(L.scratch_bytes + acc_bytes) * SCAN_WARPS : 0;
  if (smem > 48 * 1024) {
    cudaError_t e = cudaFuncSetAttribute(scan_agg_kernel, cudaFuncAttributeMaxDynamicSharedMemorySize, (int)smem);
    if (e != cudaSuccess) return e;
  }
  scan_agg_kernel<<<L.grid, SCAN_WARPS * 32, smem, L.stream>>>(L.arena, L.rec_off, order, item_begin, n_items, L.q, agg_op,
      pval, pcnt, L.gscratch, L.scratch_bytes, acc_bytes, L.use_smem, L.d_counters, L.d_err);
  return cudaGetLastError();
}
cudaError_t launch_merge_partials(const double* pval, const uint32_t* pcnt, const int64_t* gis, int n_groups, int T, int agg_op,
                                  int partial_out, double* out_val, int64_t* out_cnt, cudaStream_t s) {
  const int ktiles = (T + 31) / 32;
  if (agg_moments(agg_op)) merge_partials_kernel<MERGE_MOMENTS><<<n_groups * ktiles, 256, 0, s>>>(pval, pcnt, gis, n_groups, T, agg_op, partial_out, out_val, out_cnt);
  else if (agg_op == AGG_GROUP) merge_partials_kernel<MERGE_GROUP><<<n_groups * ktiles, 256, 0, s>>>(pval, pcnt, gis, n_groups, T, agg_op, partial_out, out_val, out_cnt);
  else merge_partials_kernel<<<n_groups * ktiles, 256, 0, s>>>(pval, pcnt, gis, n_groups, T, agg_op, partial_out, out_val, out_cnt);
  return cudaGetLastError();
}
cudaError_t launch_present(int agg_op, int64_t n, const double* vals, const int64_t* cnts, double* out, cudaStream_t s) {
  present_kernel<<<(unsigned)((n + 255) / 256), 256, 0, s>>>(agg_op, n, vals, cnts, out);
  return cudaGetLastError();
}
cudaError_t launch_topk(const double* per_series, const int32_t* order, const int64_t* group_start, int n_groups, int T, int k, int bottom,
                        double* out_val, int64_t* out_id, cudaStream_t s) {
  const int64_t n = (int64_t)n_groups * T;
  topk_kernel<<<(unsigned)((n + 127) / 128), 128, 0, s>>>(per_series, order, group_start, n_groups, T, k, bottom, out_val, out_id);
  return cudaGetLastError();
}
cudaError_t launch_iota(int32_t* a, int64_t n, cudaStream_t s) {
  iota_kernel<<<(unsigned)((n + 255) / 256), 256, 0, s>>>(a, n); return cudaGetLastError();
}
// ... 16 lines not shown
```

### filodb_b200/csrc/scan_wp.cuh

```cuda
#pragma once
#include "scan_tile.cuh"
#include "scan_wp_layout.h"

namespace filo {

#ifdef FILO_CUSIM
__device__ __forceinline__ uint32_t wp_soff(const void* p) { return (uint32_t)(reinterpret_cast<const uint8_t*>(p) - smem); }
__device__ __forceinline__ uint32_t wp_lds32(uint32_t off) { uint32_t v; std::memcpy(&v, smem + off, 4); return v; }
#else
__device__ __forceinline__ uint32_t wp_soff(const void* p) { return smem_u32(p); }
__device__ __forceinline__ uint32_t wp_lds32(uint32_t off) { uint32_t v; asm volatile("ld.shared.u32 %0, [%1];" : "=r"(v) : "r"(off)); return v; }
#endif

#if defined(FILO_WP_PROF) && !defined(FILO_CUSIM)
__device__ unsigned long long g_wp_prof[16];
#define WPROF_DECL uint32_t wpp_t0 = (uint32_t)clock(), wpp_acc[14] = {0, 0, 0, 0, 0, 0, 0, 0, 0, 0, 0, 0, 0, 0};
#define WPROF(i) { const uint32_t wpp_t1 = (uint32_t)clock(); wpp_acc[i] += wpp_t1 - wpp_t0; wpp_t0 = wpp_t1; }
#define WPROF_COUNT(i) { ++wpp_acc[i]; }
#define WPROF_FLUSH if (lane == 0) { for (int wpp_i = 0; wpp_i < 14; ++wpp_i) atomicAdd(&g_wp_prof[wpp_i], (unsigned long long)wpp_acc[wpp_i]); atomicAdd(&g_wp_prof[15], 1ull); }
#else
#define WPROF_DECL
#define WPROF(i)
#define WPROF_COUNT(i)
#define WPROF_FLUSH
// ... 59 lines not shown
    case 2: wp_block_tail<2>(pa, pb, a, b); break;
    case 3: wp_block_tail<3>(pa, pb, a, b); break;
    case 4: wp_block_tail<4>(pa, pb, a, b); break;
    case 5: wp_block_tail<5>(pa, pb, a, b); break;
    case 6: wp_block_tail<6>(pa, pb, a, b); break;
    default: wp_block_tail<7>(pa, pb, a, b); break;
  }
}

struct WpParsed {
  bool regular, have, any_raw; bool irr;
  int tslope; uint32_t toff;
  int n, cLo;
  int64_t init, end_time; int nrows, num_rows, vbytes, ng, vwire, dropped, tlen, grp_base, ngroups; uint32_t voff, w12;
};
template <bool STRICT, bool IRR = false>
__device__ __forceinline__ WpParsed wp_parse(const uint8_t* R, const QueryParams& q, bool staged, int lane) {
  const unsigned FULL = 0xffffffffu;
  WpParsed P;
  bool regular = staged;
  int n = 0, cLo = 0;
  if (staged) {
    const RecordHeader* h = reinterpret_cast<const RecordHeader*>(R);
    const ChunkEntry* Eall = reinterpret_cast<const ChunkEntry*>(R + sizeof(RecordHeader));
    const int nch = (int)h->n_chunks;
    regular = nch <= 32 && (IRR || (h->flags & REC_ALL_TS_CONST) != 0);
    const int64_t t1 = q.start - q.window, t2 = q.end;
    bool below = false, within = false;
    if (regular && lane < nch) { below = Eall[lane].end_time < t1; within = !below && Eall[lane].start_time <= t2; }
    const unsigned mb = __ballot_sync(FULL, below), mw = __ballot_sync(FULL, within);
    cLo = __ffs((int)~mb) - 1; if (cLo < 0) cLo = 32;
    const unsigned rest = cLo < 32 ? (mw >> cLo) : 0u;
    n = __ffs((int)~rest) - 1; if (n < 0) n = 32;
    if (n > WP_MAXC) regular = false;
  }
  const int c = lane;
  bool have = regular && c < n;
  int64_t init = 0, end_time = 0; int nrows = 0, num_rows = 0, vbytes = 0, ng = 0, vwire = 0, dropped = 0, tlen = 0; uint32_t voff = 0, w12 = 0;
  bool okc = true, irrc = false; int slope = 0; uint32_t toff = 0;
  if (have) {
    const ChunkEntry& e = reinterpret_cast<const ChunkEntry*>(R + sizeof(RecordHeader))[cLo + c];
    const uint8_t* tv = R + e.ts_off; const uint8_t* vv = R + e.val_off;
    const uint32_t vw4 = ld32(vv + 4);
    vwire = (int)(vw4 & 0xffff); dropped = (int)((vw4 >> 31) & 1);
    toff = e.ts_off;
    const int twire = (int)(ld32(tv + 4) & 0xffff);
    if (!IRR || twire == WIRE_DDV_CONST) { tlen = (int)ld32(tv + 8); init = (int64_t)ld64_a4(tv + 12); slope = (int)ld32(tv + 20); if (IRR && twire != WIRE_DDV_CONST) okc = false; }
    else if (twire == WIRE_DDV) {
      init = (int64_t)ld64(tv + 8); slope = (int)ld32(tv + 16); tlen = int_length(tv + 20); irrc = true;
      const int nb = (int)((ld32(tv + 24) >> 16) & 0x7f);
      if (!(nb == 2 || nb == 4 || nb == 8 || nb == 16 || nb == 32)) okc = false;
    } else okc = false;
    if (IRR && (int64_t)slope != q.step) irrc = true;
    end_time = e.end_time; num_rows = e.num_rows; voff = e.val_off;
    vbytes = (int)ld32(tv) + 4 + (int)ld32(vv) + 4;
    int vlen = 0;
    if (vwire == WIRE_XOR) { vlen = (int)ld32(vv + XOR_OFF_N); w12 = ld32(vv + XOR_OFF_NGROUPS); ng = (int)(w12 & 0xffff); if (ng != (vlen + 6) / 8) okc = false; }
    else if (vwire == WIRE_RAW64) vlen = ((int)ld32(vv) - 4) / 8;
    else okc = false;
    if ((!IRR && (int64_t)slope != q.step) || slope <= 0 || tlen <= 0 || vlen <= 0 || num_rows <= 0) okc = false;
    nrows = num_rows < tlen ? num_rows : tlen;
    if (vlen != nrows) okc = false;
    if (STRICT && end_time < init + (int64_t)(nrows - 1) * q.step) okc = false;
  }
  {
    const int64_t endp = __shfl_up_sync(FULL, end_time, 1);
    if (STRICT && have && c > 0 && !(endp < init)) okc = false;
    if (!__all_sync(FULL, okc)) regular = false;
  }
  have = have && regular;
  if (!have) { ng = 0; nrows = 0; }
  int grp_base = ng;
  { const int a0 = __shfl_sync(FULL, ng, 0), a1 = __shfl_sync(FULL, ng, 1), a2 = __shfl_sync(FULL, ng, 2), a3 = __shfl_sync(FULL, ng, 3);
    grp_base = (c > 0 ? a0 : 0) + (c > 1 ? a1 : 0) + (c > 2 ? a2 : 0);
    if (a0 + a1 + a2 + a3 > WP_MAXG) regular = false; }
  P.ngroups = __shfl_sync(FULL, grp_base + ng, WP_MAXC - 1);
  P.any_raw = __any_sync(FULL, have && vwire == WIRE_RAW64);
  P.irr = IRR && __any_sync(FULL, have && irrc); P.tslope = slope; P.toff = toff;
  P.regular = regular; P.have = have && regular; P.n = n; P.cLo = cLo; P.init = init; P.end_time = end_time; P.nrows = nrows; P.num_rows = num_rows;
  P.vbytes = vbytes; P.ng = ng; P.vwire = vwire; P.dropped = dropped; P.tlen = tlen; P.grp_base = grp_base; P.voff = voff; P.w12 = w12;
  return P;
}

struct WpNoop { __device__ __forceinline__ void operator()() const {} };
template <bool DROPS, typename RDone = WpNoop>
__device__ __forceinline__ uint32_t wp_decode(const uint8_t* R, double* V, const WpChunk* CD, uint64_t* xtab, const int dd_dst[2], const int dd_inf[2],
                                              int n, bool any_raw, int lane, TileDrops* DR, RDone r_done = RDone()) {
  uint32_t okbits = 0xffffffffu;
  uint64_t d[2][8];
#pragma unroll
  for (int jj = 0; jj < 2; ++jj) {
    const bool active = dd_inf[jj] & 1;
    const WpChunk& ch = CD[(dd_inf[jj] >> 1) & 3];
    const uint8_t* gp = R;
    if (active) gp = R + ch.grp_off + reinterpret_cast<const uint16_t*>(R + ch.tab_off)[dd_inf[jj] >> 8];
    const uint32_t mask = active ? gp[0] : 0u;
    const uint32_t hdr = gp[1];
    const uint32_t numBits = ((hdr >> 4) + 1) * 4;
    const uint32_t tz = (hdr & 0x0f) * 4;
    const uint64_t fm = (~0ull >> (64 - numBits)) << tz;
    uint32_t xb = (wp_soff(gp + 2) << 3) - tz;
    uint64_t x = 0;
#pragma unroll
    for (int i = 0; i < 8; ++i) {
      const bool on = (mask >> i) & 1u;
      const uint32_t wa = (xb >> 3) & ~3u;
      const uint32_t w0 = wp_lds32(wa), w1 = wp_lds32(wa + 4), w2 = wp_lds32(wa + 8);
      const uint32_t lo = __funnelshift_r(w0, w1, xb), hi = __funnelshift_r(w1, w2, xb);
      const uint64_t f = on ? fm : 0ull;
      x ^= (((uint64_t)hi << 32) | lo) & f;
      xb += on ? numBits : 0u;
      d[jj][i] = x;
    }
  }
  if (!any_raw) r_done();
  uint64_t i0x = d[0][7], i1x = d[1][7];
#pragma unroll
  for (int o = 1; o < 32; o <<= 1) {
    const uint64_t y0 = shfl_up_u64(i0x, o), y1 = shfl_up_u64(i1x, o);
    if (lane >= o) { i0x ^= y0; i1x ^= y1; }
  }
  const uint64_t tot0 = shfl_u64(i0x, 31);
  const uint64_t ex0 = i0x ^ d[0][7], ex1 = i1x ^ d[1][7] ^ tot0;
  xtab[lane] = ex0; xtab[32 + lane] = ex1;
  __syncwarp();
#pragma unroll
  for (int jj = 0; jj < 2; ++jj) {
    const bool active = dd_inf[jj] & 1;
    const int ci = (dd_inf[jj] >> 1) & 3;
    const WpChunk& ch = CD[ci];
    const uint64_t pre = ch.first ^ (jj ? ex1 : ex0) ^ xtab[active ? ch.grp_base : 0];
    uint64_t* dst = reinterpret_cast<uint64_t*>(V) + dd_dst[jj];
    const int t = (dd_inf[jj] >> 3) & 7;
    if (active) {
#pragma unroll
      for (int i = 0; i < 8; ++i) {
        const uint64_t b = d[jj][i] ^ pre;
        dst[i + ((t + i) >> 3)] = b;
        const uint32_t h = (uint32_t)(b >> 32);
        okbits &= h ^ (h << 1);
      }
      if ((dd_inf[jj] >> 8) == 0) { dst[t == 0 ? -2 : -1] = ch.first; const uint32_t h = (uint32_t)(ch.first >> 32); okbits &= h ^ (h << 1); }
      if (DROPS && ch.dropped) {
        const int g = dd_inf[jj] >> 8;
        const int nleft = ch.nrows - 1 - g * 8;
        double prevv = nan0(__longlong_as_double((long long)pre));
        TileDrops& D = DR[ci];
#pragma unroll
        for (int i = 0; i < 8; ++i) {
          const double cur = nan0(__longlong_as_double((long long)(d[jj][i] ^ pre)));
          if (i < nleft && cur < prevv) {
            const int at = atomicAdd(&D.n, 1);
            if (at < TILE_MAXDROP) { D.pos[at] = 1 + g * 8 + i; D.amt[at] = prevv; }
          }
          prevv = cur;
        }
      }
    }
  }
  for (int ci = 0; any_raw && ci < n; ++ci) {
    const WpChunk& ch = CD[ci];
    if (ch.wire != WIRE_RAW64) continue;
    const uint64_t* src = reinterpret_cast<const uint64_t*>(R + ch.val_off + 8);
    const bool drp = DROPS && ch.dropped;
    for (int r = lane; r < ch.nrows; r += 32) {
      const uint64_t b = src[r];
      reinterpret_cast<uint64_t*>(V)[wp_vidx(ch.rowpos + r)] = b;
      const uint32_t h = (uint32_t)(b >> 32);
      okbits &= h ^ (h << 1);
      if (drp && r > 0) {
        const double cur = nan0(__longlong_as_double((long long)b)), prevv = nan0(__longlong_as_double((long long)src[r - 1]));
        if (cur < prevv) { TileDrops& D = DR[ci]; const int at = atomicAdd(&D.n, 1); if (at < TILE_MAXDROP) { D.pos[at] = r; D.amt[at] = prevv; } }
      }
    }
  }
  if (any_raw) r_done();
  return okbits;
}

constexpr uint32_t WP_FINAL = 0, WP_RAWFIN = 1, WP_JUNC = 2, WP_GAP = 3;
__device__ __forceinline__ int wp_chunk_of(const WpChunk* CD, int n, int k) {
  int ci = -1;
  for (int c = 0; c < n; ++c) if (CD[c].nblk > 0 && k >= CD[c].kT0) ci = c;
  return ci;
}
__device__ __forceinline__ uint32_t wp_class(const WpChunk* CD, int n, int k, uint32_t& jslot) {
  const int ci = wp_chunk_of(CD, n, k);
  jslot = 0;
  if (ci < 0 || k > CD[ci].kT1) return WP_GAP;
  const WpChunk& ch = CD[ci];
  const int i = k - ch.kT0;
  if (i < ch.jzb * WP_R) { jslot = (uint32_t)(ch.joff + i) | (i < ch.hs ? 128u : 0u); return WP_JUNC; }
  return i >= ch.tb * WP_R ? WP_RAWFIN : WP_FINAL;
}
__device__ __forceinline__ int wp_rows_in(const WpChunk& x, int k, int Wr) {
  int lo = x.s0 + k; if (lo < 0) lo = 0; int hi = x.s0 + k + Wr; if (hi > x.nrows - 1) hi = x.nrows - 1;
  return hi - lo + 1;
}

__device__ __forceinline__ void wp_item(const WpChunk* CD, const WpSmem& L, int it, int items, int psi, int& pp, int& op, int& inf) {
  const bool active = it < items;
  int ci = 0;
  if (CD[1].nblk > 0 && it >= CD[1].blk0) ci = 1;
  if (CD[2].nblk > 0 && it >= CD[2].blk0) ci = 2;
  if (CD[3].nblk > 0 && it >= CD[3].blk0) ci = 3;
  const WpChunk& ch = CD[ci];
  const int b = active ? it - ch.blk0 : 0;
  const int k0 = ch.kT0 + WP_R * b;
  pp = ch.vidx0 + 9 * b;
  const bool tojz = b < ch.jzb;
  const bool raw = tojz || b >= ch.tb;
  op = tojz ? (int)WP_OFF_J + 8 * (ch.joff + WP_R * b) : (int)L.out + 8 * (k0 + ((k0 + psi) >> 3));
  int jEnd = !active ? -1 : tojz ? WP_R - 1 : ch.kT1 - k0;
  if (jEnd > WP_R - 1) jEnd = WP_R - 1;
  const int ot = tojz ? 0 : (k0 + psi) & 7;
  inf = (jEnd + 1) | ((raw ? 1 : 0) << 4) | (ot << 5) | (ci << 8) | (k0 << 10);
}

template <int FN, int NW>
__global__ void __launch_bounds__(NW * 32, 1)
scan_wp_sum_kernel(const uint8_t* __restrict__ arena, const int64_t* __restrict__ rec_off, int64_t n_series, QueryParams q,
                   double* __restrict__ out, WpSmem L, int64_t* __restrict__ fallback_list, unsigned long long* __restrict__ fallback_count,
                   unsigned long long* d_counters, int* d_err) {
  extern __shared__ __align__(128) uint8_t smem[];
  const unsigned FULL = 0xffffffffu;
  const int lane = threadIdx.x & 31, warp = threadIdx.x >> 5;
  uint8_t* wb = smem + (size_t)warp * L.per_warp;
  uint64_t* bar = reinterpret_cast<uint64_t*>(wb);
  WpChunk* CD = reinterpret_cast<WpChunk*>(wb + WP_OFF_DESC);
  uint64_t* xtab = reinterpret_cast<uint64_t*>(wb + WP_OFF_J);
  double* J = reinterpret_cast<double*>(wb + WP_OFF_J);
  const bool two = L.rec2 != 0;
  uint8_t* R = wb + WP_OFF_REC;
  double* V = reinterpret_cast<double*>(wb + L.vals);
  double* O = reinterpret_cast<double*>(wb + L.out);
  const int64_t nwarps = (int64_t)gridDim.x * (blockDim.x >> 5);
  int64_t s = (int64_t)blockIdx.x * (blockDim.x >> 5) + warp;
  if (lane == 0) { mbar_init(bar, 1); if (two) mbar_init(bar + 1, 1); mbar_fence_init(); }
  __syncwarp();

  int64_t winDur = q.inclusive ? q.window : q.window - 1; if (winDur < 0) winDur = 0;
  const double fdiv = (double)(q.inclusive ? winDur : winDur + 1), frcp = 1.0 / fdiv;
  const int64_t S0 = q.start - winDur, E0 = q.start;
  const int64_t lastEnd = q.start + (int64_t)(q.T - 1) * q.step;
  StepDiv sd; sd.init(q.step);
  const double NaNv = __longlong_as_double(0x7ff8000000000000LL);

  int64_t m_init = 0, m_end = 0; int m_nrows = -1, m_n = -1, m_wire = -1; bool m_ok = false;
  int dd_dst[2] = {0, 0}, dd_inf[2] = {0, 0}, wi_pp[2] = {0, 0}, wi_op[2] = {0, 0}, wi_inf[2] = {0, 0};
  int gz[3] = {-1, -1, -1}; bool gz_all = true;
  int p_Wr = 0, p_items = 0, p_nfull = 0, p_psi = 0; double p_rcpn = 0.0; bool p_oal = false;
  uint32_t p_cls = 0; uint64_t p_jx = 0;
  int64_t rows_scanned = 0, bytes_scanned = 0;
  uint32_t parity = 0;

  auto issue = [&](int64_t off, uint32_t sz) {
    uint64_t* b = bar + (R == wb + WP_OFF_REC ? 0 : 1);
    mbar_expect_tx(b, sz);
    tma_load_1d(R, arena + off, sz, b);
  };
  uint32_t cur_sz = 0, nb_sz = 0;
  int64_t cur_off = 0;
  if (s < n_series) { cur_off = rec_off[s]; cur_sz = (uint32_t)(rec_off[s + 1] - cur_off); }
  if (s < n_series && cur_sz <= L.rec_cap && lane == 0) issue(cur_off, cur_sz);
  if (two && s + nwarps < n_series) {
    const int64_t o1 = rec_off[s + nwarps]; nb_sz = (uint32_t)(rec_off[s + nwarps + 1] - o1);
    R = wb + L.rec2;
    if (nb_sz <= L.rec_cap && lane == 0) issue(o1, nb_sz);
    R = wb + WP_OFF_REC;
  }
  uint32_t stage = 0;
  WPROF_DECL

  for (; s < n_series; s += nwarps) {
    const int64_t sn = s + (two ? 2 : 1) * nwarps;
    int64_t nxt_off = 0; uint32_t nxt_end = 0;
    if (sn < n_series) { nxt_off = rec_off[sn]; nxt_end = (uint32_t)rec_off[sn + 1]; }
    const bool staged = cur_sz <= L.rec_cap;
    WPROF_COUNT(10)
    WPROF(9)
    if (staged) { mbar_wait(bar + stage, (parity >> stage) & 1u); parity ^= 1u << stage; }
    WPROF(0)
    const WpParsed P = wp_parse<true>(R, q, staged, lane);
    const uint32_t nxt_sz = nxt_end - (uint32_t)nxt_off;
    WPROF(1)
    bool regular = P.regular;
    const bool have = P.have; const int n = P.n, c = lane;
    const int64_t init = P.init, end_time = P.end_time;
    const int nrows = P.nrows, num_rows = P.num_rows, vbytes = P.vbytes, ng = P.ng, vwire = P.vwire, grp_base = P.grp_base, ngroups = P.ngroups;
    const uint32_t voff = P.voff, w12 = P.w12; const bool any_raw = P.any_raw;
    const bool samec = !(c < n) || (init == m_init && nrows == m_nrows && end_time == m_end && vwire == m_wire);
    const bool same_all = __all_sync(FULL, samec);
    const bool same = m_ok && n == m_n && same_all;
    if (regular && !same) {
      WPROF_COUNT(11)
      m_init = init; m_end = end_time; m_nrows = nrows; m_n = n; m_wire = vwire; m_ok = false;
      int64_t s0 = 0, e0 = 0;
      if (have) { s0 = sd.ceil_div(S0 - init); e0 = sd.floor_div(E0 - init); }
      const int Wr = (int)(e0 - s0);
      int64_t kT0 = -e0; if (kT0 < 0) kT0 = 0;
      int64_t kT1 = (int64_t)(nrows - 1) - s0; if (kT1 > q.T - 1) kT1 = q.T - 1;
      const bool touch = have && kT0 <= kT1;
      if (!touch) { kT0 = 0x3fffffff; kT1 = -1; }
      const int Wr0 = __shfl_sync(FULL, Wr, 0);
      bool okp = !have || Wr == Wr0;
      if (Wr0 < 8 || (uint32_t)Wr0 + 1 > L.jcap) okp = false;
      const unsigned tm = __ballot_sync(FULL, touch) & 0xfu;
      if (tm != 0) { const unsigned lowbit = tm & (0u - tm); const unsigned filled = tm + lowbit; if ((filled & (filled - 1)) != 0) okp = false; }
      const int64_t kT1p = __shfl_up_sync(FULL, kT1, 1), kT1pp = __shfl_up_sync(FULL, kT1, 2), kT0n = __shfl_down_sync(FULL, kT0, 1);
      const bool prev_t = c > 0 && ((tm >> (c - 1)) & 1u), next_t = c + 1 < WP_MAXC && ((tm >> (c + 1)) & 1u);
      if (touch && c >= 2 && ((tm >> (c - 2)) & 1u) && !(kT1pp < kT0)) okp = false;
      int64_t ownLo = kT0, ownHi = kT1;
      if (touch && prev_t && kT1p + 1 > ownLo) ownLo = kT1p + 1;
      if (touch && next_t && kT0n - 1 < ownHi) ownHi = kT0n - 1;
      const int hs = touch ? (int)(ownLo - kT0) : 0;
      const int nblk = touch ? (int)((kT1 - kT0 + WP_R) / WP_R) : 0;
      const int jzb = (hs + WP_R - 1) / WP_R;
      const int tb = (touch && ownHi < kT1) ? (int)((ownHi + 1 - kT0) / WP_R) : nblk;
      if (touch && jzb > tb) okp = false;
      int blk0, items, joff, jtot;
      { const int a0 = __shfl_sync(FULL, nblk, 0), a1 = __shfl_sync(FULL, nblk, 1), a2 = __shfl_sync(FULL, nblk, 2), a3 = __shfl_sync(FULL, nblk, 3);
        blk0 = (c > 0 ? a0 : 0) + (c > 1 ? a1 : 0) + (c > 2 ? a2 : 0); items = a0 + a1 + a2 + a3; }
      { const int z = jzb * WP_R;
        const int a0 = __shfl_sync(FULL, z, 0), a1 = __shfl_sync(FULL, z, 1), a2 = __shfl_sync(FULL, z, 2), a3 = __shfl_sync(FULL, z, 3);
        joff = (c > 0 ? a0 : 0) + (c > 1 ? a1 : 0) + (c > 2 ? a2 : 0); jtot = a0 + a1 + a2 + a3; }
      if ((uint32_t)jtot > L.jcap) okp = false;
      if (L.alias && items > 64) okp = false;
      const int fr = touch ? (int)(s0 + kT0) : 0;
      int rowpos = 0;
      {
        int base = 0;
#pragma unroll
        for (int cc = 0; cc < WP_MAXC; ++cc) {
          int x;
          if (cc == 0) { x = fr < 0 ? -fr : ((8 - (fr & 7)) & 7); }
          else { x = base + ((-(base + fr)) & 7); }
          if (c == cc) rowpos = x;
          const int nb = __shfl_sync(FULL, x + nrows + Wr0, cc);
          base = nb;
        }
      }
      const int pend = __shfl_sync(FULL, rowpos + nrows, n > 0 ? n - 1 : 0) + Wr0 + 8;
      if ((uint32_t)(pend + (pend >> 3) + 2) > L.vcap) okp = false;
      if (!__all_sync(FULL, okp)) regular = false;
      if (regular) {
        if (c < WP_MAXC) {
          WpChunk& d = CD[c];
          d.kT0 = (int)kT0; d.kT1 = (int)kT1; d.ownLo = (int)ownLo; d.ownHi = (int)ownHi; d.blk0 = blk0; d.nblk = nblk;
          d.vidx0 = wp_vidx(rowpos + fr); d.rowpos = rowpos; d.nrows = nrows; d.s0 = (int)s0; d.e0 = (int)e0; d.joff = joff; d.hs = hs; d.jzb = jzb; d.tb = tb;
        }
        { const int first_t = tm ? __ffs((int)tm) - 1 : 0;
          p_psi = (-(int)__shfl_sync(FULL, (int)(touch ? kT0 : 0), first_t)) & 7;
          p_oal = __all_sync(FULL, !touch || (((int)kT0 + p_psi) & 7) == 0); }
        p_Wr = Wr0; p_items = items; p_nfull = Wr0 + 1; p_rcpn = 1.0 / (double)(Wr0 + 1);
        __syncwarp();
        {
          int tot = 0;
          gz[0] = gz[1] = gz[2] = -1;
          for (int g = 0; g <= n; ++g) {
            const int g0 = g == 0 ? 0 : CD[g - 1].rowpos + CD[g - 1].nrows;
            const int g1 = g == n ? pend : CD[g].rowpos;
#pragma unroll
            for (int u = 0; u < 3; ++u) { const int i = u * 32 + lane - tot; if (i >= 0 && i < g1 - g0) gz[u] = wp_vidx(g0 + i); }
            tot += g1 - g0;
          }
          gz_all = tot <= 96;
        }
        {
          uint32_t cls = 0; uint64_t jx = 0; int nj = 0;
#pragma unroll 1
          for (int m = 0; m < 16 && lane + 32 * m < q.T; ++m) {
            uint32_t js;
            const uint32_t code = wp_class(CD, n, lane + 32 * m, js);
            cls |= code << (2 * m);
            if (code == WP_JUNC) { jx |= (uint64_t)js << (8 * nj); ++nj; }
          }
          p_cls = cls; p_jx = jx;
        }
        {
          const int gb1 = __shfl_sync(FULL, have ? grp_base : 0x7fffffff, 1), gb2 = __shfl_sync(FULL, have ? grp_base : 0x7fffffff, 2),
                    gb3 = __shfl_sync(FULL, have ? grp_base : 0x7fffffff, 3);
#pragma unroll
          for (int jj = 0; jj < 2; ++jj) {
            const int slot = jj * 32 + lane;
            const bool active = slot < ngroups;
            const int ci = active ? (slot >= gb1 ? 1 : 0) + (slot >= gb2 ? 1 : 0) + (slot >= gb3 ? 1 : 0) : 0;
            const int gbc = ci == 0 ? 0 : ci == 1 ? gb1 : ci == 2 ? gb2 : gb3;
            const int g = active ? slot - gbc : 0;
            const int pq = CD[ci].rowpos + 1 + g * 8;
            dd_dst[jj] = wp_vidx(pq);
            dd_inf[jj] = (active ? 1 : 0) | (ci << 1) | ((pq & 7) << 3) | (g << 8);
          }
#pragma unroll
          for (int X = 0; X < 2; ++X) wp_item(CD, L, X * 32 + lane, items, p_psi, wi_pp[X], wi_op[X], wi_inf[X]);
        }
        m_ok = true;
      }
    }
    WPROF(2)
    if (!regular) {
      WPROF_COUNT(12)
      if (lane == 0) { const unsigned long long slot = atomicAdd(fallback_count, 1ull); fallback_list[slot] = s; }
      __syncwarp();
      if (sn < n_series && nxt_sz <= L.rec_cap && lane == 0) issue(nxt_off, nxt_sz);
      if (two) { cur_sz = nb_sz; nb_sz = nxt_sz; stage ^= 1u; R = wb + (stage ? L.rec2 : WP_OFF_REC); } else cur_sz = nxt_sz;
      continue;
    }
    if (c < WP_MAXC) {
      WpChunk& d = CD[c];
      d.grp_base = have ? grp_base : 0x7fffffff; d.ng = ng; d.wire = vwire; d.val_off = voff; d.dropped = P.dropped;
      if (have && vwire == WIRE_XOR) { const uint32_t po = w12 >> 16; d.first = ld64(R + voff + po); d.grp_off = voff + po + 8; d.tab_off = voff + XOR_OFF_GROUPTAB; }
      else { d.first = have ? ld64(R + voff + 8) : 0ull; d.grp_off = 0; d.tab_off = 0; }
    }
    int cnt_rows = 0, cnt_bytes = 0;
    { const int64_t endp = __shfl_up_sync(FULL, end_time, 1);
      if (have && !(c > 0 && !(endp < lastEnd))) { cnt_rows = num_rows; cnt_bytes = vbytes; } }
#pragma unroll
    for (int o = 1; o < WP_MAXC; o <<= 1) { cnt_rows += __shfl_xor_sync(FULL, cnt_rows, o); cnt_bytes += __shfl_xor_sync(FULL, cnt_bytes, o); }
    __syncwarp();
    WPROF(3)
    auto rec_done = [&]() {
      __syncwarp();
      if (sn < n_series && nxt_sz <= L.rec_cap && lane == 0) issue(nxt_off, nxt_sz);
    };
    const uint32_t okbits = wp_decode<false>(R, V, CD, xtab, dd_dst, dd_inf, n, any_raw, lane, nullptr, rec_done);
    const bool vals_ok = __all_sync(FULL, (okbits >> 30) & 1u);
    __syncwarp();
    if (two) { cur_sz = nb_sz; nb_sz = nxt_sz; stage ^= 1u; R = wb + (stage ? L.rec2 : WP_OFF_REC); } else cur_sz = nxt_sz;
    WPROF(4)
    if (gz_all) {
#pragma unroll
      for (int u = 0; u < 3; ++u) if (gz[u] >= 0) V[gz[u]] = 0.0;
    } else {
      const int pend = CD[n - 1].rowpos + CD[n - 1].nrows + p_Wr + 8;
      for (int g = 0; g <= n; ++g) {
        const int g0 = g == 0 ? 0 : CD[g - 1].rowpos + CD[g - 1].nrows;
        const int g1 = g == n ? pend : CD[g].rowpos;
        for (int pz = g0 + lane; pz < g1; pz += 32) V[wp_vidx(pz)] = 0.0;
      }
    }
    WPROF(5)
    if (!vals_ok) {
      WPROF_COUNT(13)
      if (lane == 0) { const unsigned long long slot = atomicAdd(fallback_count, 1ull); fallback_list[slot] = s; }
      __syncwarp();
      continue;
    }
    if (lane == 0) { rows_scanned += cnt_rows; bytes_scanned += cnt_bytes; }
    __syncwarp();
    const int psi = p_psi;
    auto oidx = [&](int k) -> int { return k + ((k + psi) >> 3); };
    {
      const int Wr = p_Wr;
      for (int it0 = 0; it0 < p_items; it0 += 64) {
        int ipp[2], iop[2], iinf[2];
#pragma unroll
        for (int X = 0; X < 2; ++X) {
          if (it0 == 0) { ipp[X] = wi_pp[X]; iop[X] = wi_op[X]; iinf[X] = wi_inf[X]; }
          else wp_item(CD, L, it0 + X * 32 + lane, p_items, psi, ipp[X], iop[X], iinf[X]);
        }
        const double* pp[2]; double* op[2]; int jEnd[2], ot[2]; bool rawm[2];
#pragma unroll
        for (int X = 0; X < 2; ++X) {
          pp[X] = V + ipp[X]; op[X] = reinterpret_cast<double*>(wb + iop[X]);
          jEnd[X] = (iinf[X] & 15) - 1; rawm[X] = (iinf[X] >> 4) & 1; ot[X] = (iinf[X] >> 5) & 7;
        }
        double a[WP_R], bb[WP_R];
        wp_block_pair(pp[0], pp[1], Wr, a, bb);
        __syncwarp();
#pragma unroll
        for (int X = 0; X < 2; ++X) {
          const double dv = rawm[X] ? 1.0 : fdiv, rc = rawm[X] ? 1.0 : frcp, sc = rawm[X] ? 1.0 : 1000.0;
#pragma unroll
          for (int j = 0; j < WP_R; ++j) {
            const double raw = X ? bb[j] : a[j];
            int nn = 1;
            if (FN == FN_AVG || FN == FN_COUNT) {
              const WpChunk& ch = CD[(iinf[X] >> 8) & 3];
              int lo = ch.s0 + (iinf[X] >> 10) + j; const int hi0 = lo + Wr; if (lo < 0) lo = 0;
              const int hi = hi0 > ch.nrows - 1 ? ch.nrows - 1 : hi0;
              nn = hi - lo + 1;
            }
            const double fin = wp_finish<FN>(raw, nn, dv, rc, sc, p_nfull, p_rcpn, rawm[X]);
            if (X) bb[j] = fin; else a[j] = fin;
          }
        }
        if (p_oal) {
#pragma unroll
          for (int j = 0; j < WP_R; ++j) { if (j <= jEnd[0]) op[0][j] = a[j]; if (j <= jEnd[1]) op[1][j] = bb[j]; }
        } else {
#pragma unroll
          for (int j = 0; j < WP_R; ++j) {
            if (j <= jEnd[0]) op[0][j + ((ot[0] + j) >> 3)] = a[j];
            if (j <= jEnd[1]) op[1][j + ((ot[1] + j) >> 3)] = bb[j];
          }
        }
      }
      __syncwarp();
      WPROF(6)
      double* gp = out + (size_t)s * q.T + lane;
      const double* sp = O + oidx(lane);
      auto fin = [&](double o, uint32_t code, uint32_t js, int k) -> double {
        double v = o;
        if (code == WP_JUNC) { const double jv = J[js & 127u]; v = (js & 128u) ? o + jv : jv; }
        double r;
        if (FN == FN_COUNT) r = v;
        else {
          int nn = 1;
          if (FN == FN_AVG && (code == WP_RAWFIN || code == WP_JUNC)) {
            const int ci = wp_chunk_of(CD, n, k);
            nn = wp_rows_in(CD[ci], k, Wr);
            if (code == WP_JUNC && (js & 128u)) nn += wp_rows_in(CD[ci - 1], k, Wr);
          }
          r = wp_finish<FN>(v, nn, fdiv, frcp, 1000.0, p_nfull, p_rcpn, false);
        }
        return code == WP_FINAL ? o : code == WP_GAP ? NaNv : r;
      };
      uint32_t cls = p_cls; uint64_t jx = p_jx;
      auto fin_m = [&](double o, int k) -> double {
        const uint32_t code = cls & 3u, js = (uint32_t)jx & 0xffu;
        cls >>= 2;
        if (code == WP_JUNC) jx >>= 8;
        return fin(o, code, js, k);
      };
      int k = lane, iters = (q.T - lane + 31) >> 5;
      int rest = iters > 16 ? iters - 16 : 0;
      if (rest) iters = 16;
      for (; iters >= 4; iters -= 4, gp += 128, sp += 144, k += 128) {
        const double v0 = sp[0], v1 = sp[36], v2 = sp[72], v3 = sp[108];
        const double r0 = fin_m(v0, k), r1 = fin_m(v1, k + 32), r2 = fin_m(v2, k + 64), r3 = fin_m(v3, k + 96);
        wp_store_result(gp, r0); wp_store_result(gp + 32, r1); wp_store_result(gp + 64, r2); wp_store_result(gp + 96, r3);
      }
      for (; iters > 0; --iters, gp += 32, sp += 36, k += 32) wp_store_result(gp, fin_m(*sp, k));
      for (; rest > 0; --rest, gp += 32, sp += 36, k += 32) {
        uint32_t js;
        const uint32_t code = wp_class(CD, n, k, js);
        wp_store_result(gp, fin(*sp, code, js, k));
      }
    }
    __syncwarp();
    WPROF(7)
  }
  WPROF(9)
  WPROF_FLUSH
  if (lane == 0) {
    if (rows_scanned | bytes_scanned) { atomicAdd(&d_counters[0], (unsigned long long)rows_scanned); atomicAdd(&d_counters[1], (unsigned long long)bytes_scanned); }
  }
}

}
```

### filodb_b200/csrc/scan_wp_layout.h

```cpp
#pragma once
#include <stdint.h>
#include "filo_record.h"
#include "scan_params.h"
#include "scan_tile_layout.h"
namespace filo {
constexpr int WP_MAXC = 4;
constexpr int WP_MAXG = 64;
constexpr int WP_R = 8;
constexpr int WP_MAX_WARPS = 16;
constexpr int WP_MAX_WARPS_ALIAS = 20;

struct WpChunk {
  uint64_t first;
  int32_t kT0, kT1;
  int32_t ownLo, ownHi;
  int32_t blk0, nblk;
  int32_t vidx0;
  int32_t rowpos;
  int32_t nrows, s0, e0;
  int32_t grp_base, ng, wire;
  uint32_t grp_off, tab_off, val_off;
  int32_t joff, hs;
  int32_t jzb, tb;
  int32_t dropped;
};
static_assert(sizeof(WpChunk) == 96, "WpChunk");

constexpr uint32_t WP_OFF_DESC = 16, WP_OFF_J = WP_OFF_DESC + WP_MAXC * 96, WP_J_DOUBLES = 128, WP_OFF_REC = WP_OFF_J + WP_J_DOUBLES * 8;
struct WpSmem {
  uint32_t desc, jbuf, rec, vals, out, per_warp;
  uint32_t rec_cap, vcap , jcap , ocap ;
  uint32_t warps;
  uint32_t alias;
  uint32_t rec2;
};
FILO_HD inline WpSmem wp_layout(uint32_t max_rec_bytes, uint32_t max_rows, uint32_t max_chunks, uint32_t T, uint32_t wrows, bool alias, bool two_rec = false) {
  WpSmem L;
  if (max_chunks > (uint32_t)WP_MAXC) max_chunks = WP_MAXC;
  L.rec_cap = align_up(max_rec_bytes + 16, 16);
  const uint32_t P = max_rows + (max_chunks + 1) * (wrows + 7) + 16;
  L.vcap = align_up(P + P / 8 + 2, 2);
  L.jcap = WP_J_DOUBLES;
  (void)wrows;
  L.ocap = align_up(T + T / 8 + 4, 2);
  if (alias && L.vcap < L.ocap) L.vcap = L.ocap;
  static_assert(sizeof(WpChunk) == 96, "WP_OFF_J");
  uint32_t o = WP_OFF_REC;
  L.desc = WP_OFF_DESC; L.jbuf = WP_OFF_J;
  L.rec = o; o += L.rec_cap;
  L.rec2 = 0;
  if (two_rec) { L.rec2 = o; o += L.rec_cap; }
  L.vals = o; o += L.vcap * 8;
  if (alias) L.out = L.vals; else { L.out = o; o += L.ocap * 8; }
  L.per_warp = align_up(o, 16);
  L.warps = 0;
  L.alias = alias ? 1u : 0u;
  return L;
}
FILO_HD inline uint32_t wp_max_items(uint32_t max_chunks, uint32_t T, uint32_t wrows) {
  if (max_chunks > (uint32_t)WP_MAXC) max_chunks = WP_MAXC;
  if (max_chunks == 0) max_chunks = 1;
  return (T + (max_chunks - 1) * (wrows - 1) + 7 * max_chunks) / 8;
}

constexpr int WP_CTR_MAX_WARPS = 20;
struct TileCtr {
  double dTS, thr, half, endpart, sI, ratio0, skipC;
  int32_t dropped, pad;
};
constexpr int TILE_MAXDROP = 8;
constexpr int TILE_CTR_TABMAX = 64;
struct TileCtrTab { double sI, thr, half, rcpSI; };
struct TileDrops {
  int32_t n, pos[TILE_MAXDROP], pad[3];
  double amt[TILE_MAXDROP];
};
struct WpCtrChunk {
  int64_t init, end_time;
  int32_t nrows, s0, e0, rowpos;
  int32_t kA, kB;
  int32_t kA2, kB2;
  TileCtr kc;
};
static_assert(sizeof(WpCtrChunk) == 112, "WpCtrChunk");

struct WpCtrSmem {
  uint32_t vals, kc, acc, nbad, per_warp, tab ;
  uint32_t rec_cap, vcap , warps, agg;
  uint32_t tsr;
};
constexpr uint32_t WP_OFF_DROPS = WP_OFF_J + 64 * 8;
static_assert(WP_OFF_DROPS + WP_MAXC * sizeof(TileDrops) <= WP_OFF_REC, "drops fit in front of the record");
FILO_HD inline WpCtrSmem wp_ctr_layout(uint32_t max_rec_bytes, uint32_t max_rows, uint32_t max_chunks, uint32_t T, bool agg, bool irr = false,
                                       bool moments = false) {
  WpCtrSmem L;
  if (max_chunks > (uint32_t)WP_MAXC) max_chunks = WP_MAXC;
  L.rec_cap = align_up(max_rec_bytes + 16, 16);
  const uint32_t P = max_rows + 8 * max_chunks + 8;
  L.vcap = align_up(P + P / 8 + 2, 2);
  uint32_t o = WP_OFF_REC + L.rec_cap;
  L.vals = o; o += L.vcap * 8;
  L.kc = o; o += (uint32_t)(WP_MAXC * sizeof(WpCtrChunk));
  L.tsr = 0;
  if (irr) { L.tsr = o; o += align_up(P * 4, 16); }
  L.acc = o; L.nbad = o;
  if (agg) { o += T * 8; L.nbad = o; o += align_up(T * 2, 16); }
  if (agg && moments) o += T * 8;
  L.per_warp = align_up(o, 16);
  L.tab = 0; L.warps = 0; L.agg = agg ? 1u : 0u;
// ... 10 lines not shown
```

Before: 152.9 billion.

## Precompute per-series shape directory to skip per-record parse in warp scan

Adds a per-table series directory built at load time that holds each record's offset, size and a shape id, found by hashing chunk timestamps, row counts and wire headers into a dedup table. The warp-per-series scan kernel reads this directory instead of rec_off and reuses its cached per-shape plan whenever consecutive series share a shape id, which avoids the full per-record parse and cross-lane shape comparison. It adds a build pass at load/append time and per-batch in the streaming path, plus a 16-byte directory read per series. Correctness depends on shape equality covering every field the plan uses.

```diff
diff --git a/filodb_b200/csrc/capi.cu b/filodb_b200/csrc/capi.cu
--- a/filodb_b200/csrc/capi.cu
+++ b/filodb_b200/csrc/capi.cu
@@ -60,6 +60,7 @@
   bool any_drop = true;
   uint8_t* d_arena = nullptr;
   int64_t* d_rec_off = nullptr;
+  WpDirEnt* d_dir = nullptr;
   int32_t n_groups = 1;
   bool grouped = false;
   int32_t* d_order = nullptr;
@@ -144,7 +145,7 @@
 void filo_table_free(filo_ctx* ctx, filo_table* t) {
   if (!t) return;
   if (ctx) cudaSetDevice(ctx->device);
-  cudaFree(t->d_arena); cudaFree(t->d_rec_off); cudaFree(t->d_order); cudaFree(t->d_group_start);
+  cudaFree(t->d_arena); cudaFree(t->d_rec_off); cudaFree(t->d_dir); cudaFree(t->d_order); cudaFree(t->d_group_start);
   cudaFree(t->d_gis); cudaFree(t->d_item_begin); cudaFree(t->d_hist_tops);
   delete t;
 }
@@ -232,7 +233,22 @@
   return FILO_OK;
 }
 
+static int32_t build_series_dir(filo_ctx* ctx, filo_table* t) {
+  cudaStream_t s = ctx->stream;
+  cudaFree(t->d_dir); t->d_dir = nullptr;
+  if (t->n_series <= 0) return FILO_OK;
+  int32_t* slots = nullptr;
+  CUDA_TRY(ctx, cudaMalloc(&t->d_dir, (size_t)t->n_series * sizeof(WpDirEnt)));
+  CUDA_TRY(ctx, cudaMallocAsync((void**)&slots, (size_t)wp_dir_slots(t->n_series) * 4, s));
+  const cudaError_t e = launch_series_dir(t->d_arena, t->d_rec_off, t->n_series, slots, t->d_dir, s);
+  cudaFreeAsync(slots, s);
+  CUDA_TRY(ctx, e);
+  CUDA_TRY(ctx, cudaStreamSynchronize(s));
+  return FILO_OK;
+}
 int32_t filo_internal_finish_table(filo_ctx* ctx, filo_table* t, const int32_t* d_group_ids, int32_t n_groups) {
+  const int32_t rc = build_series_dir(ctx, t);
+  if (rc != FILO_OK) return rc;
   return build_groups(ctx, t, d_group_ids, n_groups);
 }
 filo_table* filo_internal_new_table() { return new filo_table(); }
@@ -554,7 +570,7 @@
     CUDA_TRY(ctx, cudaMalloc(&d_gid, (size_t)n_series * 4));
     CUDA_TRY(ctx, cudaMemcpy(d_gid, group_ids, (size_t)n_series * 4, cudaMemcpyHostToDevice));
   }
-  int32_t rc = build_groups(ctx, t, d_gid, group_ids ? n_groups : 1);
+  int32_t rc = filo_internal_finish_table(ctx, t, d_gid, group_ids ? n_groups : 1);
   cudaFree(d_gid);
   if (rc) { filo_table_free(ctx, t); return rc; }
   *out = t;
@@ -690,7 +706,7 @@
   t->arena_bytes = arena_bytes + (S + 1) * 8;
   t->max_rec_bytes = st[0]; t->max_rows = (int32_t)st[1]; t->max_chunks = (int32_t)st[2];
   t->any_nonconst_ts = t->any_nonconst_ts || (d->n_chunks > 0 && d->any_nonconst_ts); t->any_drop = t->any_drop || d->any_drop;
-  return FILO_OK;
+  return build_series_dir(ctx, t);
 }
 extern "C" int32_t filo_table_append(filo_ctx* ctx, filo_table* t, const int32_t* n_chunks, const uint64_t* chunk_info_addrs, int32_t ts_col, int32_t val_col) {
   try { return filo_table_append_impl(ctx, t, n_chunks, chunk_info_addrs, ts_col, val_col); }
@@ -837,6 +853,7 @@
   int64_t launches = 0;
   uint8_t* gscratch = nullptr;
   ScanLaunch L{t->d_arena, t->d_rec_off, t->n_series, q, nullptr, 0, 0, d_counters, d_err, 1, s};
+  L.dir = t->d_dir;
   uint32_t rec_cap_used = 0;
   if (use_v2) {
     const size_t cta_smem = per_warp2 * FAST_WARPS + 1024;
@@ -1314,8 +1331,17 @@
     view.n_series = nb; view.d_arena = sl.d_in; view.d_rec_off = sl.d_off; view.max_rows = tot.maxrows; view.max_chunks = tot.maxch;
     view.max_rec_bytes = tot.max_rec; view.any_nonconst_ts = !(tot.f_and & REC_ALL_TS_CONST); view.any_drop = (tot.f_or & REC_ANY_DROP) != 0;
     view.schema_flags = schema_flags; view.n_groups = 1; view.grouped = false;
+    {
+      int32_t* slots = nullptr;
+      ce = cudaMallocAsync((void**)&view.d_dir, (size_t)nb * sizeof(WpDirEnt), sl.stream);
+      if (ce == cudaSuccess) ce = cudaMallocAsync((void**)&slots, (size_t)wp_dir_slots(nb) * 4, sl.stream);
+      if (ce == cudaSuccess) ce = launch_series_dir(view.d_arena, view.d_rec_off, nb, slots, view.d_dir, sl.stream);
+      if (slots) cudaFreeAsync(slots, sl.stream);
+      if (ce != cudaSuccess) { if (view.d_dir) cudaFreeAsync(view.d_dir, sl.stream); rc = fail(ctx, FILO_ERR_CUDA, std::string("scan directory: ") + cudaGetErrorString(ce)); break; }
+    }
     rc = query_device_impl(ctx, &view, fn, start, step, end, window, FILO_AGG_NONE, 0, 0, sl.d_out, nullptr, sl.stream, nullptr,
                            reinterpret_cast<AsyncSink*>(sl.h_sink));
+    cudaFreeAsync(view.d_dir, sl.stream); view.d_dir = nullptr;
     if (rc != FILO_OK) break;
     if (trace_path) cudaEventRecord(trace.back().ev[2], sl.stream);
     ce = cudaMemcpyAsync(out_values + (size_t)B.s0 * T, sl.d_out, (size_t)nb * T * 8, cudaMemcpyDeviceToHost, sl.stream);
@@ -1394,6 +1420,7 @@
   cudaEvent_t& e0 = evp.e0; cudaEvent_t& e1 = evp.e1;
   const int64_t work = fused ? t->n_items : t->n_series;
   ScanLaunch L{t->d_arena, t->d_rec_off, t->n_series, q, nullptr, 0, 0, d_counters, d_err, 1, s};
+  L.dir = t->d_dir;
   const int ctas_per_sm = (int)std::max<size_t>(1, (size_t)(228 * 1024) / (smem + 2048));
   L.grid = (int)std::max<int64_t>(1, std::min<int64_t>(work, (int64_t)ctx->sm_count * ctas_per_sm));
   const int64_t rows = fused ? t->n_groups : t->n_series;
diff --git a/filodb_b200/csrc/kernels.h b/filodb_b200/csrc/kernels.h
--- a/filodb_b200/csrc/kernels.h
+++ b/filodb_b200/csrc/kernels.h
@@ -21,6 +21,7 @@
 }
 #include "scan_params.h"
 #include "scan_tile_layout.h"
+#include "scan_wp_layout.h"
 namespace filo {
 
 struct ScanLaunch {
@@ -30,6 +31,7 @@
   unsigned long long* d_counters; int* d_err;
   int grid; cudaStream_t stream;
   const int64_t* list = nullptr; const unsigned long long* list_count = nullptr;
+  const WpDirEnt* dir = nullptr;
 };
 
 cudaError_t launch_scan_series(const ScanLaunch& L, double* out);
@@ -48,6 +50,7 @@
 cudaError_t launch_topk(const double* per_series, const int32_t* order, const int64_t* group_start, int n_groups, int T, int k, int bottom,
                         double* out_val, int64_t* out_id, cudaStream_t s);
 struct WpSmem;
+cudaError_t launch_series_dir(const uint8_t* arena, const int64_t* rec_off, int64_t n_series, int32_t* slots, WpDirEnt* dir, cudaStream_t s);
 cudaError_t launch_scan_wp(const ScanLaunch& L, double* out, const WpSmem& W, int64_t* fallback_list, unsigned long long* fallback_count);
 struct WpCtrSmem;
 cudaError_t launch_scan_wp_ctr(const ScanLaunch& L, double* out, const WpCtrSmem& W, int64_t* fallback_list, unsigned long long* fallback_count);
diff --git a/filodb_b200/csrc/scan_kernels.cu b/filodb_b200/csrc/scan_kernels.cu
--- a/filodb_b200/csrc/scan_kernels.cu
+++ b/filodb_b200/csrc/scan_kernels.cu
@@ -1,4 +1,5 @@
 #include <cuda_runtime.h>
+#include <algorithm>
 #include <stdint.h>
 #define FILO_DEV_ERR_TS_WIRE 1
 #define FILO_DEV_ERR_VAL_WIRE 2
@@ -466,12 +467,22 @@
   return moments ? launch_tile_any<true, true>(L, nullptr, T, fallback_list, fallback_count, A)
                  : launch_tile_any<true>(L, nullptr, T, fallback_list, fallback_count, A);
 }
+cudaError_t launch_series_dir(const uint8_t* arena, const int64_t* rec_off, int64_t n_series, int32_t* slots, WpDirEnt* dir, cudaStream_t s) {
+  if (n_series <= 0) return cudaSuccess;
+  if (n_series > INT32_MAX) return cudaErrorInvalidValue;
+  const uint32_t nslots = wp_dir_slots(n_series);
+  cudaError_t e = cudaMemsetAsync(slots, 0xff, (size_t)nslots * 4, s);
+  if (e != cudaSuccess) return e;
+  const int64_t blocks = std::min<int64_t>((n_series + 255) / 256, 1 << 16);
+  wp_dir_kernel<<<(unsigned)blocks, 256, 0, s>>>(arena, rec_off, n_series, slots, nslots - 1, dir);
+  return cudaGetLastError();
+}
 template <int FN, int NW>
 static cudaError_t launch_wp_nw(const ScanLaunch& L, double* out, const WpSmem& W, int64_t* fallback_list, unsigned long long* fallback_count) {
   const size_t smem = (size_t)W.per_warp * W.warps;
   cudaError_t e = cudaFuncSetAttribute(scan_wp_sum_kernel<FN, NW>, cudaFuncAttributeMaxDynamicSharedMemorySize, (int)smem);
   if (e != cudaSuccess) return e;
-  scan_wp_sum_kernel<FN, NW><<<L.grid, W.warps * 32, smem, L.stream>>>(L.arena, L.rec_off, L.n_series, L.q, out, W, fallback_list, fallback_count, L.d_counters, L.d_err);
+  scan_wp_sum_kernel<FN, NW><<<L.grid, W.warps * 32, smem, L.stream>>>(L.arena, L.dir, L.n_series, L.q, out, W, fallback_list, fallback_count, L.d_counters, L.d_err);
   return cudaGetLastError();
 }
 template <int FN>
@@ -480,6 +491,7 @@
   return launch_wp_nw<FN, WP_MAX_WARPS_ALIAS>(L, out, W, fallback_list, fallback_count);
 }
 cudaError_t launch_scan_wp(const ScanLaunch& L, double* out, const WpSmem& W, int64_t* fallback_list, unsigned long long* fallback_count) {
+  if (!L.dir) return cudaErrorInvalidValue;
   switch (L.q.fn) {
     case FN_RATE: return launch_wp_fn<FN_RATE>(L, out, W, fallback_list, fallback_count);
     case FN_AVG: return launch_wp_fn<FN_AVG>(L, out, W, fallback_list, fallback_count);
diff --git a/filodb_b200/csrc/scan_wp.cuh b/filodb_b200/csrc/scan_wp.cuh
--- a/filodb_b200/csrc/scan_wp.cuh
+++ b/filodb_b200/csrc/scan_wp.cuh
@@ -165,6 +165,57 @@
   return P;
 }
 
+__device__ __forceinline__ bool wp_shape_never(const uint8_t* r) {
+  const RecordHeader* h = reinterpret_cast<const RecordHeader*>(r);
+  return !(h->flags & REC_ALL_TS_CONST) || (h->flags & REC_HIST) || h->n_chunks == 0 || h->n_chunks > 32;
+}
+constexpr int WP_SHAPE_CW = 13;
+__device__ __forceinline__ void wp_shape_chunk(const uint8_t* r, uint32_t c, uint32_t w[WP_SHAPE_CW]) {
+  const ChunkEntry& e = reinterpret_cast<const ChunkEntry*>(r + sizeof(RecordHeader))[c];
+  const uint8_t* tv = r + e.ts_off; const uint8_t* vv = r + e.val_off;
+  w[0] = (uint32_t)e.start_time; w[1] = (uint32_t)(e.start_time >> 32); w[2] = (uint32_t)e.end_time; w[3] = (uint32_t)(e.end_time >> 32);
+  w[4] = (uint32_t)e.num_rows;
+  for (int k = 0; k < 5; ++k) w[5 + k] = ld32(tv + 4 + 4 * k);
+  const uint32_t vw = ld32(vv + 4);
+  w[10] = vw;
+  if ((int)(vw & 0xffff) == WIRE_XOR) { w[11] = ld32(vv + XOR_OFF_N); w[12] = ld32(vv + XOR_OFF_NGROUPS) & 0xffffu; }
+  else { w[11] = ld32(vv); w[12] = 0; }
+}
+__device__ __forceinline__ uint32_t wp_shape_hash(const uint8_t* r) {
+  const RecordHeader* h = reinterpret_cast<const RecordHeader*>(r);
+  uint32_t hv = 2166136261u;
+  auto mix = [&](uint32_t x) { hv = (hv ^ x) * 16777619u; hv ^= hv >> 15; };
+  mix(h->n_chunks); mix(h->n_rows); mix(h->flags);
+  for (uint32_t c = 0; c < h->n_chunks; ++c) { uint32_t w[WP_SHAPE_CW]; wp_shape_chunk(r, c, w); for (int k = 0; k < WP_SHAPE_CW; ++k) mix(w[k]); }
+#ifdef FILO_WP_DIR_WEAK_HASH
+  hv &= 3u;
+#endif
+  return hv;
+}
+__device__ __forceinline__ bool wp_shape_same(const uint8_t* a, const uint8_t* b) {
+  const RecordHeader* ha = reinterpret_cast<const RecordHeader*>(a);
+  const RecordHeader* hb = reinterpret_cast<const RecordHeader*>(b);
+  if (ha->n_chunks != hb->n_chunks || ha->n_rows != hb->n_rows || ha->flags != hb->flags) return false;
+  for (uint32_t c = 0; c < ha->n_chunks; ++c) {
+    uint32_t wa[WP_SHAPE_CW], wb[WP_SHAPE_CW];
+    wp_shape_chunk(a, c, wa); wp_shape_chunk(b, c, wb);
+    for (int k = 0; k < WP_SHAPE_CW; ++k) if (wa[k] != wb[k]) return false;
+  }
+  return true;
+}
+__device__ __forceinline__ void wp_dir_series(const uint8_t* arena, const int64_t* rec_off, int64_t i, int32_t* slots, uint32_t mask, WpDirEnt* dir) {
+  const int64_t o = rec_off[i];
+  const uint8_t* r = arena + o;
+  WpDirEnt e; e.off = o; e.bytes = (uint32_t)(rec_off[i + 1] - o); e.shape = WP_SHAPE_NONE;
+  if (!wp_shape_never(r))
+    for (uint32_t hs = wp_shape_hash(r) & mask;; hs = (hs + 1) & mask) {
+      const int32_t prev = atomicCAS(&slots[hs], -1, (int32_t)i);
+      if (prev < 0) { e.shape = (int32_t)i; break; }
+      if (wp_shape_same(r, arena + rec_off[prev])) { e.shape = prev; break; }
+    }
+  dir[i] = e;
+}
+
 struct WpNoop { __device__ __forceinline__ void operator()() const {} };
 template <bool DROPS, typename RDone = WpNoop>
 __device__ __forceinline__ uint32_t wp_decode(const uint8_t* R, double* V, const WpChunk* CD, uint64_t* xtab, const int dd_dst[2], const int dd_inf[2],
@@ -302,7 +353,7 @@
 
 template <int FN, int NW>
 __global__ void __launch_bounds__(NW * 32, 1)
-scan_wp_sum_kernel(const uint8_t* __restrict__ arena, const int64_t* __restrict__ rec_off, int64_t n_series, QueryParams q,
+scan_wp_sum_kernel(const uint8_t* __restrict__ arena, const WpDirEnt* __restrict__ dir, int64_t n_series, QueryParams q,
                    double* __restrict__ out, WpSmem L, int64_t* __restrict__ fallback_list, unsigned long long* __restrict__ fallback_count,
                    unsigned long long* d_counters, int* d_err) {
   extern __shared__ __align__(128) uint8_t smem[];
@@ -329,7 +380,8 @@
   StepDiv sd; sd.init(q.step);
   const double NaNv = __longlong_as_double(0x7ff8000000000000LL);
 
-  int64_t m_init = 0, m_end = 0; int m_nrows = -1, m_n = -1, m_wire = -1; bool m_ok = false;
+  int32_t m_shape = WP_SHAPE_NONE; bool m_ok = false;
+  int p_n = 0, p_cLo = 0, p_cnt_rows = 0; bool p_any_raw = false, p_xor = false, p_cnt = false;
   int dd_dst[2] = {0, 0}, dd_inf[2] = {0, 0}, wi_pp[2] = {0, 0}, wi_op[2] = {0, 0}, wi_inf[2] = {0, 0};
   int gz[3] = {-1, -1, -1}; bool gz_all = true;
   int p_Wr = 0, p_items = 0, p_nfull = 0, p_psi = 0; double p_rcpn = 0.0; bool p_oal = false;
@@ -342,14 +394,20 @@
     mbar_expect_tx(b, sz);
     tma_load_1d(R, arena + off, sz, b);
   };
-  uint32_t cur_sz = 0, nb_sz = 0;
-  int64_t cur_off = 0;
-  if (s < n_series) { cur_off = rec_off[s]; cur_sz = (uint32_t)(rec_off[s + 1] - cur_off); }
-  if (s < n_series && cur_sz <= L.rec_cap && lane == 0) issue(cur_off, cur_sz);
+  auto entry = [&](int64_t i, int64_t& off, uint32_t& sz) -> int32_t {
+    const int4 v = *reinterpret_cast<const int4*>(dir + i);
+    off = (int64_t)(((uint64_t)(uint32_t)v.y << 32) | (uint32_t)v.x); sz = (uint32_t)v.z;
+    return sz <= L.rec_cap ? v.w : WP_SHAPE_NONE;
+  };
+  int32_t cur_sh = WP_SHAPE_NONE, nb_sh = WP_SHAPE_NONE;
+  int64_t cur_off = 0; uint32_t cur_sz = 0;
+  if (s < n_series) cur_sh = entry(s, cur_off, cur_sz);
+  if (cur_sh != WP_SHAPE_NONE && lane == 0) issue(cur_off, cur_sz);
   if (two && s + nwarps < n_series) {
-    const int64_t o1 = rec_off[s + nwarps]; nb_sz = (uint32_t)(rec_off[s + nwarps + 1] - o1);
+    int64_t o1; uint32_t sz1;
+    nb_sh = entry(s + nwarps, o1, sz1);
     R = wb + L.rec2;
-    if (nb_sz <= L.rec_cap && lane == 0) issue(o1, nb_sz);
+    if (nb_sh != WP_SHAPE_NONE && lane == 0) issue(o1, sz1);
     R = wb + WP_OFF_REC;
   }
   uint32_t stage = 0;
@@ -357,159 +415,168 @@
 
   for (; s < n_series; s += nwarps) {
     const int64_t sn = s + (two ? 2 : 1) * nwarps;
-    int64_t nxt_off = 0; uint32_t nxt_end = 0;
-    if (sn < n_series) { nxt_off = rec_off[sn]; nxt_end = (uint32_t)rec_off[sn + 1]; }
-    const bool staged = cur_sz <= L.rec_cap;
+    int64_t nxt_off = 0; uint32_t nxt_sz = 0; int32_t nxt_sh = WP_SHAPE_NONE;
+    if (sn < n_series) nxt_sh = entry(sn, nxt_off, nxt_sz);
+    const bool staged = cur_sh != WP_SHAPE_NONE;
+    const int c = lane;
     WPROF_COUNT(10)
     WPROF(9)
     if (staged) { mbar_wait(bar + stage, (parity >> stage) & 1u); parity ^= 1u << stage; }
     WPROF(0)
-    const WpParsed P = wp_parse<true>(R, q, staged, lane);
-    const uint32_t nxt_sz = nxt_end - (uint32_t)nxt_off;
-    WPROF(1)
-    bool regular = P.regular;
-    const bool have = P.have; const int n = P.n, c = lane;
-    const int64_t init = P.init, end_time = P.end_time;
-    const int nrows = P.nrows, num_rows = P.num_rows, vbytes = P.vbytes, ng = P.ng, vwire = P.vwire, grp_base = P.grp_base, ngroups = P.ngroups;
-    const uint32_t voff = P.voff, w12 = P.w12; const bool any_raw = P.any_raw;
-    const bool samec = !(c < n) || (init == m_init && nrows == m_nrows && end_time == m_end && vwire == m_wire);
-    const bool same_all = __all_sync(FULL, samec);
-    const bool same = m_ok && n == m_n && same_all;
-    if (regular && !same) {
+    if (staged && cur_sh != m_shape) {
       WPROF_COUNT(11)
-      m_init = init; m_end = end_time; m_nrows = nrows; m_n = n; m_wire = vwire; m_ok = false;
-      int64_t s0 = 0, e0 = 0;
-      if (have) { s0 = sd.ceil_div(S0 - init); e0 = sd.floor_div(E0 - init); }
-      const int Wr = (int)(e0 - s0);
-      int64_t kT0 = -e0; if (kT0 < 0) kT0 = 0;
-      int64_t kT1 = (int64_t)(nrows - 1) - s0; if (kT1 > q.T - 1) kT1 = q.T - 1;
-      const bool touch = have && kT0 <= kT1;
-      if (!touch) { kT0 = 0x3fffffff; kT1 = -1; }
-      const int Wr0 = __shfl_sync(FULL, Wr, 0);
-      bool okp = !have || Wr == Wr0;
-      if (Wr0 < 8 || (uint32_t)Wr0 + 1 > L.jcap) okp = false;
-      const unsigned tm = __ballot_sync(FULL, touch) & 0xfu;
-      if (tm != 0) { const unsigned lowbit = tm & (0u - tm); const unsigned filled = tm + lowbit; if ((filled & (filled - 1)) != 0) okp = false; }
-      const int64_t kT1p = __shfl_up_sync(FULL, kT1, 1), kT1pp = __shfl_up_sync(FULL, kT1, 2), kT0n = __shfl_down_sync(FULL, kT0, 1);
-      const bool prev_t = c > 0 && ((tm >> (c - 1)) & 1u), next_t = c + 1 < WP_MAXC && ((tm >> (c + 1)) & 1u);
-      if (touch && c >= 2 && ((tm >> (c - 2)) & 1u) && !(kT1pp < kT0)) okp = false;
-      int64_t ownLo = kT0, ownHi = kT1;
-      if (touch && prev_t && kT1p + 1 > ownLo) ownLo = kT1p + 1;
-      if (touch && next_t && kT0n - 1 < ownHi) ownHi = kT0n - 1;
-      const int hs = touch ? (int)(ownLo - kT0) : 0;
-      const int nblk = touch ? (int)((kT1 - kT0 + WP_R) / WP_R) : 0;
-      const int jzb = (hs + WP_R - 1) / WP_R;
-      const int tb = (touch && ownHi < kT1) ? (int)((ownHi + 1 - kT0) / WP_R) : nblk;
-      if (touch && jzb > tb) okp = false;
-      int blk0, items, joff, jtot;
-      { const int a0 = __shfl_sync(FULL, nblk, 0), a1 = __shfl_sync(FULL, nblk, 1), a2 = __shfl_sync(FULL, nblk, 2), a3 = __shfl_sync(FULL, nblk, 3);
-        blk0 = (c > 0 ? a0 : 0) + (c > 1 ? a1 : 0) + (c > 2 ? a2 : 0); items = a0 + a1 + a2 + a3; }
-      { const int z = jzb * WP_R;
-        const int a0 = __shfl_sync(FULL, z, 0), a1 = __shfl_sync(FULL, z, 1), a2 = __shfl_sync(FULL, z, 2), a3 = __shfl_sync(FULL, z, 3);
-        joff = (c > 0 ? a0 : 0) + (c > 1 ? a1 : 0) + (c > 2 ? a2 : 0); jtot = a0 + a1 + a2 + a3; }
-      if ((uint32_t)jtot > L.jcap) okp = false;
-      if (L.alias && items > 64) okp = false;
-      const int fr = touch ? (int)(s0 + kT0) : 0;
-      int rowpos = 0;
-      {
-        int base = 0;
-#pragma unroll
-        for (int cc = 0; cc < WP_MAXC; ++cc) {
-          int x;
-          if (cc == 0) { x = fr < 0 ? -fr : ((8 - (fr & 7)) & 7); }
-          else { x = base + ((-(base + fr)) & 7); }
-          if (c == cc) rowpos = x;
-          const int nb = __shfl_sync(FULL, x + nrows + Wr0, cc);
-          base = nb;
+      const WpParsed P = wp_parse<true>(R, q, true, lane);
+      m_shape = cur_sh; m_ok = false;
+      bool regular = P.regular;
+      const bool have = P.have; const int n = P.n;
+      const int64_t init = P.init, end_time = P.end_time;
+      const int nrows = P.nrows, ng = P.ng, grp_base = P.grp_base, ngroups = P.ngroups;
+      if (regular) {
+        int64_t s0 = 0, e0 = 0;
+        if (have) { s0 = sd.ceil_div(S0 - init); e0 = sd.floor_div(E0 - init); }
+        const int Wr = (int)(e0 - s0);
+        int64_t kT0 = -e0; if (kT0 < 0) kT0 = 0;
+        int64_t kT1 = (int64_t)(nrows - 1) - s0; if (kT1 > q.T - 1) kT1 = q.T - 1;
+        const bool touch = have && kT0 <= kT1;
+        if (!touch) { kT0 = 0x3fffffff; kT1 = -1; }
+        const int Wr0 = __shfl_sync(FULL, Wr, 0);
+        bool okp = !have || Wr == Wr0;
+        if (Wr0 < 8 || (uint32_t)Wr0 + 1 > L.jcap) okp = false;
+        const unsigned tm = __ballot_sync(FULL, touch) & 0xfu;
+        if (tm != 0) { const unsigned lowbit = tm & (0u - tm); const unsigned filled = tm + lowbit; if ((filled & (filled - 1)) != 0) okp = false; }
+        const int64_t kT1p = __shfl_up_sync(FULL, kT1, 1), kT1pp = __shfl_up_sync(FULL, kT1, 2), kT0n = __shfl_down_sync(FULL, kT0, 1);
+        const bool prev_t = c > 0 && ((tm >> (c - 1)) & 1u), next_t = c + 1 < WP_MAXC && ((tm >> (c + 1)) & 1u);
+        if (touch && c >= 2 && ((tm >> (c - 2)) & 1u) && !(kT1pp < kT0)) okp = false;
+        int64_t ownLo = kT0, ownHi = kT1;
+        if (touch && prev_t && kT1p + 1 > ownLo) ownLo = kT1p + 1;
+        if (touch && next_t && kT0n - 1 < ownHi) ownHi = kT0n - 1;
+        const int hs = touch ? (int)(ownLo - kT0) : 0;
+        const int nblk = touch ? (int)((kT1 - kT0 + WP_R) / WP_R) : 0;
+        const int jzb = (hs + WP_R - 1) / WP_R;
+        const int tb = (touch && ownHi < kT1) ? (int)((ownHi + 1 - kT0) / WP_R) : nblk;
+        if (touch && jzb > tb) okp = false;
+        int blk0, items, joff, jtot;
+        { const int a0 = __shfl_sync(FULL, nblk, 0), a1 = __shfl_sync(FULL, nblk, 1), a2 = __shfl_sync(FULL, nblk, 2), a3 = __shfl_sync(FULL, nblk, 3);
+          blk0 = (c > 0 ? a0 : 0) + (c > 1 ? a1 : 0) + (c > 2 ? a2 : 0); items = a0 + a1 + a2 + a3; }
+        { const int z = jzb * WP_R;
+          const int a0 = __shfl_sync(FULL, z, 0), a1 = __shfl_sync(FULL, z, 1), a2 = __shfl_sync(FULL, z, 2), a3 = __shfl_sync(FULL, z, 3);
+          joff = (c > 0 ? a0 : 0) + (c > 1 ? a1 : 0) + (c > 2 ? a2 : 0); jtot = a0 + a1 + a2 + a3; }
+        if ((uint32_t)jtot > L.jcap) okp = false;
+        if (L.alias && items > 64) okp = false;
+        const int fr = touch ? (int)(s0 + kT0) : 0;
+        int rowpos = 0;
+        {
+          int base = 0;
+#pragma unroll
+          for (int cc = 0; cc < WP_MAXC; ++cc) {
+            int x;
+            if (cc == 0) { x = fr < 0 ? -fr : ((8 - (fr & 7)) & 7); }
+            else { x = base + ((-(base + fr)) & 7); }
+            if (c == cc) rowpos = x;
+            const int nb = __shfl_sync(FULL, x + nrows + Wr0, cc);
+            base = nb;
+          }
+        }
+        const int pend = __shfl_sync(FULL, rowpos + nrows, n > 0 ? n - 1 : 0) + Wr0 + 8;
+        if ((uint32_t)(pend + (pend >> 3) + 2) > L.vcap) okp = false;
+        if (!__all_sync(FULL, okp)) regular = false;
+        if (regular) {
+          if (c < WP_MAXC) {
+            WpChunk& d = CD[c];
+            d.kT0 = (int)kT0; d.kT1 = (int)kT1; d.ownLo = (int)ownLo; d.ownHi = (int)ownHi; d.blk0 = blk0; d.nblk = nblk;
+            d.vidx0 = wp_vidx(rowpos + fr); d.rowpos = rowpos; d.nrows = nrows; d.s0 = (int)s0; d.e0 = (int)e0; d.joff = joff; d.hs = hs; d.jzb = jzb; d.tb = tb;
+            d.grp_base = have ? grp_base : 0x7fffffff; d.ng = ng; d.wire = P.vwire; d.dropped = P.dropped;
+            d.first = 0; d.val_off = 0; d.grp_off = 0; d.tab_off = 0;
+          }
+          { const int first_t = tm ? __ffs((int)tm) - 1 : 0;
+            p_psi = (-(int)__shfl_sync(FULL, (int)(touch ? kT0 : 0), first_t)) & 7;
+            p_oal = __all_sync(FULL, !touch || (((int)kT0 + p_psi) & 7) == 0); }
+          p_Wr = Wr0; p_items = items; p_nfull = Wr0 + 1; p_rcpn = 1.0 / (double)(Wr0 + 1);
+          __syncwarp();
+          {
+            int tot = 0;
+            gz[0] = gz[1] = gz[2] = -1;
+            for (int g = 0; g <= n; ++g) {
+              const int g0 = g == 0 ? 0 : CD[g - 1].rowpos + CD[g - 1].nrows;
+              const int g1 = g == n ? pend : CD[g].rowpos;
+#pragma unroll
+              for (int u = 0; u < 3; ++u) { const int i = u * 32 + lane - tot; if (i >= 0 && i < g1 - g0) gz[u] = wp_vidx(g0 + i); }
+              tot += g1 - g0;
+            }
+            gz_all = tot <= 96;
+          }
+          {
+            uint32_t cls = 0; uint64_t jx = 0; int nj = 0;
+#pragma unroll 1
+            for (int m = 0; m < 16 && lane + 32 * m < q.T; ++m) {
+              uint32_t js;
+              const uint32_t code = wp_class(CD, n, lane + 32 * m, js);
+              cls |= code << (2 * m);
+              if (code == WP_JUNC) { jx |= (uint64_t)js << (8 * nj); ++nj; }
+            }
+            p_cls = cls; p_jx = jx;
+          }
+          {
+            const int gb1 = __shfl_sync(FULL, have ? grp_base : 0x7fffffff, 1), gb2 = __shfl_sync(FULL, have ? grp_base : 0x7fffffff, 2),
+                      gb3 = __shfl_sync(FULL, have ? grp_base : 0x7fffffff, 3);
+#pragma unroll
+            for (int jj = 0; jj < 2; ++jj) {
+              const int slot = jj * 32 + lane;
+              const bool active = slot < ngroups;
+              const int ci = active ? (slot >= gb1 ? 1 : 0) + (slot >= gb2 ? 1 : 0) + (slot >= gb3 ? 1 : 0) : 0;
+              const int gbc = ci == 0 ? 0 : ci == 1 ? gb1 : ci == 2 ? gb2 : gb3;
+              const int g = active ? slot - gbc : 0;
+              const int pq = CD[ci].rowpos + 1 + g * 8;
+              dd_dst[jj] = wp_vidx(pq);
+              dd_inf[jj] = (active ? 1 : 0) | (ci << 1) | ((pq & 7) << 3) | (g << 8);
+            }
+#pragma unroll
+            for (int X = 0; X < 2; ++X) wp_item(CD, L, X * 32 + lane, items, p_psi, wi_pp[X], wi_op[X], wi_inf[X]);
+          }
+          p_n = n; p_cLo = P.cLo; p_any_raw = P.any_raw; p_xor = have && P.vwire == WIRE_XOR;
+          { const int64_t endp = __shfl_up_sync(FULL, end_time, 1);
+            p_cnt = have && !(c > 0 && !(endp < lastEnd));
+            int r = p_cnt ? P.num_rows : 0;
+#pragma unroll
+            for (int o = 1; o < WP_MAXC; o <<= 1) r += __shfl_xor_sync(FULL, r, o);
+            p_cnt_rows = r; }
+          m_ok = true;
         }
       }
-      const int pend = __shfl_sync(FULL, rowpos + nrows, n > 0 ? n - 1 : 0) + Wr0 + 8;
-      if ((uint32_t)(pend + (pend >> 3) + 2) > L.vcap) okp = false;
-      if (!__all_sync(FULL, okp)) regular = false;
-      if (regular) {
-        if (c < WP_MAXC) {
-          WpChunk& d = CD[c];
-          d.kT0 = (int)kT0; d.kT1 = (int)kT1; d.ownLo = (int)ownLo; d.ownHi = (int)ownHi; d.blk0 = blk0; d.nblk = nblk;
-          d.vidx0 = wp_vidx(rowpos + fr); d.rowpos = rowpos; d.nrows = nrows; d.s0 = (int)s0; d.e0 = (int)e0; d.joff = joff; d.hs = hs; d.jzb = jzb; d.tb = tb;
-        }
-        { const int first_t = tm ? __ffs((int)tm) - 1 : 0;
-          p_psi = (-(int)__shfl_sync(FULL, (int)(touch ? kT0 : 0), first_t)) & 7;
-          p_oal = __all_sync(FULL, !touch || (((int)kT0 + p_psi) & 7) == 0); }
-        p_Wr = Wr0; p_items = items; p_nfull = Wr0 + 1; p_rcpn = 1.0 / (double)(Wr0 + 1);
-        __syncwarp();
-        {
-          int tot = 0;
-          gz[0] = gz[1] = gz[2] = -1;
-          for (int g = 0; g <= n; ++g) {
-            const int g0 = g == 0 ? 0 : CD[g - 1].rowpos + CD[g - 1].nrows;
-            const int g1 = g == n ? pend : CD[g].rowpos;
-#pragma unroll
-            for (int u = 0; u < 3; ++u) { const int i = u * 32 + lane - tot; if (i >= 0 && i < g1 - g0) gz[u] = wp_vidx(g0 + i); }
-            tot += g1 - g0;
-          }
-          gz_all = tot <= 96;
-        }
-        {
-          uint32_t cls = 0; uint64_t jx = 0; int nj = 0;
-#pragma unroll 1
-          for (int m = 0; m < 16 && lane + 32 * m < q.T; ++m) {
-            uint32_t js;
-            const uint32_t code = wp_class(CD, n, lane + 32 * m, js);
-            cls |= code << (2 * m);
-            if (code == WP_JUNC) { jx |= (uint64_t)js << (8 * nj); ++nj; }
-          }
-          p_cls = cls; p_jx = jx;
-        }
-        {
-          const int gb1 = __shfl_sync(FULL, have ? grp_base : 0x7fffffff, 1), gb2 = __shfl_sync(FULL, have ? grp_base : 0x7fffffff, 2),
-                    gb3 = __shfl_sync(FULL, have ? grp_base : 0x7fffffff, 3);
-#pragma unroll
-          for (int jj = 0; jj < 2; ++jj) {
-            const int slot = jj * 32 + lane;
-            const bool active = slot < ngroups;
-            const int ci = active ? (slot >= gb1 ? 1 : 0) + (slot >= gb2 ? 1 : 0) + (slot >= gb3 ? 1 : 0) : 0;
-            const int gbc = ci == 0 ? 0 : ci == 1 ? gb1 : ci == 2 ? gb2 : gb3;
-            const int g = active ? slot - gbc : 0;
-            const int pq = CD[ci].rowpos + 1 + g * 8;
-            dd_dst[jj] = wp_vidx(pq);
-            dd_inf[jj] = (active ? 1 : 0) | (ci << 1) | ((pq & 7) << 3) | (g << 8);
-          }
-#pragma unroll
-          for (int X = 0; X < 2; ++X) wp_item(CD, L, X * 32 + lane, items, p_psi, wi_pp[X], wi_op[X], wi_inf[X]);
-        }
-        m_ok = true;
-      }
     }
     WPROF(2)
-    if (!regular) {
+    if (!staged || !m_ok) {
       WPROF_COUNT(12)
       if (lane == 0) { const unsigned long long slot = atomicAdd(fallback_count, 1ull); fallback_list[slot] = s; }
       __syncwarp();
-      if (sn < n_series && nxt_sz <= L.rec_cap && lane == 0) issue(nxt_off, nxt_sz);
-      if (two) { cur_sz = nb_sz; nb_sz = nxt_sz; stage ^= 1u; R = wb + (stage ? L.rec2 : WP_OFF_REC); } else cur_sz = nxt_sz;
+      if (nxt_sh != WP_SHAPE_NONE && lane == 0) issue(nxt_off, nxt_sz);
+      if (two) { cur_sh = nb_sh; nb_sh = nxt_sh; stage ^= 1u; R = wb + (stage ? L.rec2 : WP_OFF_REC); } else cur_sh = nxt_sh;
       continue;
     }
-    if (c < WP_MAXC) {
+    const int n = p_n; const bool any_raw = p_any_raw;
+    int cnt_bytes = 0;
+    if (c < n) {
+      const ChunkEntry& e = reinterpret_cast<const ChunkEntry*>(R + sizeof(RecordHeader))[p_cLo + c];
+      const uint32_t voff = e.val_off;
+      const uint8_t* vv = R + voff;
       WpChunk& d = CD[c];
-      d.grp_base = have ? grp_base : 0x7fffffff; d.ng = ng; d.wire = vwire; d.val_off = voff; d.dropped = P.dropped;
-      if (have && vwire == WIRE_XOR) { const uint32_t po = w12 >> 16; d.first = ld64(R + voff + po); d.grp_off = voff + po + 8; d.tab_off = voff + XOR_OFF_GROUPTAB; }
-      else { d.first = have ? ld64(R + voff + 8) : 0ull; d.grp_off = 0; d.tab_off = 0; }
-    }
-    int cnt_rows = 0, cnt_bytes = 0;
-    { const int64_t endp = __shfl_up_sync(FULL, end_time, 1);
-      if (have && !(c > 0 && !(endp < lastEnd))) { cnt_rows = num_rows; cnt_bytes = vbytes; } }
-#pragma unroll
-    for (int o = 1; o < WP_MAXC; o <<= 1) { cnt_rows += __shfl_xor_sync(FULL, cnt_rows, o); cnt_bytes += __shfl_xor_sync(FULL, cnt_bytes, o); }
+      d.val_off = voff;
+      if (p_xor) { const uint32_t po = ld32(vv + XOR_OFF_NGROUPS) >> 16; d.first = ld64(vv + po); d.grp_off = voff + po + 8; d.tab_off = voff + XOR_OFF_GROUPTAB; }
+      else d.first = ld64(vv + 8);
+      if (p_cnt) cnt_bytes = (int)ld32(R + e.ts_off) + 4 + (int)ld32(vv) + 4;
+    }
+#pragma unroll
+    for (int o = 1; o < WP_MAXC; o <<= 1) cnt_bytes += __shfl_xor_sync(FULL, cnt_bytes, o);
     __syncwarp();
     WPROF(3)
     auto rec_done = [&]() {
       __syncwarp();
-      if (sn < n_series && nxt_sz <= L.rec_cap && lane == 0) issue(nxt_off, nxt_sz);
+      if (nxt_sh != WP_SHAPE_NONE && lane == 0) issue(nxt_off, nxt_sz);
     };
     const uint32_t okbits = wp_decode<false>(R, V, CD, xtab, dd_dst, dd_inf, n, any_raw, lane, nullptr, rec_done);
     const bool vals_ok = __all_sync(FULL, (okbits >> 30) & 1u);
     __syncwarp();
-    if (two) { cur_sz = nb_sz; nb_sz = nxt_sz; stage ^= 1u; R = wb + (stage ? L.rec2 : WP_OFF_REC); } else cur_sz = nxt_sz;
+    if (two) { cur_sh = nb_sh; nb_sh = nxt_sh; stage ^= 1u; R = wb + (stage ? L.rec2 : WP_OFF_REC); } else cur_sh = nxt_sh;
     WPROF(4)
     if (gz_all) {
 #pragma unroll
@@ -529,7 +596,7 @@
       __syncwarp();
       continue;
     }
-    if (lane == 0) { rows_scanned += cnt_rows; bytes_scanned += cnt_bytes; }
+    if (lane == 0) { rows_scanned += p_cnt_rows; bytes_scanned += cnt_bytes; }
     __syncwarp();
     const int psi = p_psi;
     auto oidx = [&](int k) -> int { return k + ((k + psi) >> 3); };
@@ -631,4 +698,21 @@
   }
 }
 
-}
+__global__ void wp_dir_kernel(const uint8_t* __restrict__ arena, const int64_t* __restrict__ rec_off, int64_t n_series, int32_t* __restrict__ slots,
+                              uint32_t mask, WpDirEnt* __restrict__ dir) {
+  for (int64_t i = (int64_t)blockIdx.x * blockDim.x + threadIdx.x; i < n_series; i += (int64_t)gridDim.x * blockDim.x)
+    wp_dir_series(arena, rec_off, i, slots, mask, dir);
+}
+
+#ifdef FILO_CUSIM
+template <int FN, int NW>
+void scan_wp_sum_kernel(const uint8_t* arena, const int64_t* rec_off, int64_t n_series, QueryParams q, double* out, WpSmem L,
+                        int64_t* fallback_list, unsigned long long* fallback_count, unsigned long long* d_counters, int* d_err) {
+  std::vector<int32_t> slots(wp_dir_slots(n_series), -1);
+  std::vector<WpDirEnt> dir((size_t)n_series + 1);
+  for (int64_t i = 0; i < n_series; ++i) wp_dir_series(arena, rec_off, i, slots.data(), (uint32_t)slots.size() - 1, dir.data());
+  scan_wp_sum_kernel<FN, NW>(arena, dir.data(), n_series, q, out, L, fallback_list, fallback_count, d_counters, d_err);
+}
+#endif
+
+}
diff --git a/filodb_b200/csrc/scan_wp_layout.h b/filodb_b200/csrc/scan_wp_layout.h
--- a/filodb_b200/csrc/scan_wp_layout.h
+++ b/filodb_b200/csrc/scan_wp_layout.h
@@ -25,6 +25,15 @@
   int32_t dropped;
 };
 static_assert(sizeof(WpChunk) == 96, "WpChunk");
+
+constexpr int32_t WP_SHAPE_NONE = -1;
+struct WpDirEnt {
+  int64_t off;
+  uint32_t bytes;
+  int32_t shape;
+};
+static_assert(sizeof(WpDirEnt) == 16, "WpDirEnt");
+inline uint32_t wp_dir_slots(int64_t n) { uint32_t m = 64; while ((int64_t)m < 2 * n) m <<= 1; return m; }
 
 constexpr uint32_t WP_OFF_DESC = 16, WP_OFF_J = WP_OFF_DESC + WP_MAXC * 96, WP_J_DOUBLES = 128, WP_OFF_REC = WP_OFF_J + WP_J_DOUBLES * 8;
 struct WpSmem {
```

New measurement: 156.5 billion, median of 6. +2.4%, better.
